# google-research/corenet

Measured on AMD Instinct MI355X. Metric: voxels/sec fwd+bwd @128^3, higher is better.
Workload: dtype bf16x3 (the convolutions of decoder stages 3-6 and the encoder's 3x3 convolutions -- forward of stages 4-5, data gradient of all -- multiply operands split into two bf16 terms: three bf16 MFMAs per product, fp32 accumulation, 16 mantissa bits, ~3e-6 relative per layer; tensors, everything else and t

## Files before the change

corenet_amd/_lib.py:

```python
from __future__ import annotations

import ctypes as C
import os
from typing import Optional

import torch as t

_HERE = os.path.dirname(os.path.abspath(__file__))
TOOLS_LIB_PATH = os.path.join(os.path.dirname(_HERE), "tools", "_build", "libcorenet_hip_tools.so")
PROBE_LIB_PATH = os.path.join(os.path.dirname(_HERE), "tools", "_build", "libcrn_probe.so")
LIB_PATH = os.environ.get("CORENET_HIP_LIB", TOOLS_LIB_PATH if os.environ.get("CRN_TOOLS_LIB") == "1" else
                          os.path.join(_HERE, "lib", "libcorenet_hip.so"))

c_i32p = C.POINTER(C.c_int32)
c_f32p = C.c_void_p
vp = C.c_void_p
i64 = C.c_int64
i32 = C.c_int
f32 = C.c_float
sz = C.c_size_t


class CrnTapBoxes(C.Structure):
  _fields_ = [("n_groups", C.c_int32), ("c_groups", C.c_int32), ("n_box", (C.c_int8 * 6) * 8),
              ("c_box", (C.c_int8 * 6) * 8)]


class CrnView(C.Structure):
  _fields_ = [("base", vp), ("B", C.c_int32), ("C", C.c_int32), ("D", C.c_int32),
              ("H", C.c_int32), ("W", C.c_int32), ("sB", i64), ("sC", i64),
              ("chan_off", vp), ("sD", C.c_int32), ("sH", C.c_int32), ("sW", C.c_int32)]


class CrnConvPlan(C.Structure):
  _fields_ = [(n, C.c_int32) for n in ("path", "msub", "nsub", "xstage", "dystage", "forced", "cc", "td", "th", "tw", "mw",
                                        "splits", "chunks", "vec_store", "balanced", "lds_bytes", "lds_budget")]


class CrnBf3Plan(C.Structure):
  _fields_ = [(n, C.c_int32) for n in ("kind", "nsub", "xmode", "ng", "slabs", "td", "th", "tw", "splits", "chunks", "per_split",
                                        "vec_store", "mode", "rowskip", "half_last", "lead", "n_groups", "c_groups", "nparts",
                                        "dmode", "tpw", "twt", "pipe", "inherit", "boxskip", "lds_bytes")]


BF3_KINDS = {0: "plain", 1: "half", 2: "ws"}
PLAN_PATHS = {1: "dense_cols", 2: "dense_rows", 3: "dense_wgrad", 4: "pointwise", 5: "generic"}


class CrnInTransform(C.Structure):
  _fields_ = [("scale", vp), ("shift", vp), ("pre_relu", C.c_int32), ("post_relu", C.c_int32)]


class CrnBnBwdFuse(C.Structure):
  _fields_ = [("x", vp), ("sB_x", i64), ("saved", vp), ("pre_relu", C.c_int32), ("ws", vp), ("ws_bytes", sz),
              ("dsum", vp), ("ndsum", C.c_int32), ("nparts", C.c_int32)]


class HipError(RuntimeError):
  pass


_SIGS = {
    "crn_conv_fwd": [C.POINTER(CrnView), C.POINTER(CrnInTransform), vp, i32, vp, i32,
                     C.POINTER(CrnView), i32, i32, i32, i32, i32, i32, i32, i32, vp, vp],
    "crn_conv_fwd_plan": [C.POINTER(CrnView), C.POINTER(CrnInTransform), vp, i32, vp, i32,
                          C.POINTER(CrnView), i32, i32, i32, i32, i32, i32, i32, i32, vp, C.POINTER(CrnConvPlan)],
    "crn_conv_wgrad_plan": [C.POINTER(CrnView), C.POINTER(CrnInTransform), C.POINTER(CrnView), vp, i32,
                            i32, i32, i32, i32, i32, i32, i32, vp, C.POINTER(CrnConvPlan)],
    "crn_conv_fwd_bf3": [C.POINTER(CrnView), C.POINTER(CrnInTransform), vp, i32, vp, i32,
                         C.POINTER(CrnView), i32, i32, i32, i32, i32, i32, i32, vp, vp],
    "crn_conv_fwd_bf3_slabs": [C.POINTER(CrnView), C.POINTER(CrnInTransform), vp, i32, vp, i32,
                               C.POINTER(CrnView), i32, i32, i32, i32, i32, i32, i32, vp, vp],
    "crn_conv_fwd_bf3_slabs_bnbwd": [C.POINTER(CrnView), C.POINTER(CrnInTransform), vp, i32, vp, i32,
                                     C.POINTER(CrnView), i32, i32, i32, i32, i32, i32, i32, vp, C.POINTER(CrnBnBwdFuse), vp],
    "crn_conv_fwd_bf3_slabs_stats": [C.POINTER(CrnView), C.POINTER(CrnInTransform), vp, i32, vp, i32,
                                     C.POINTER(CrnView), i32, i32, i32, i32, i32, i32, i32, vp, i32, vp, sz, C.POINTER(C.c_int), vp],
    "crn_batch_renorm_bwd_apply": [vp, i64, vp, i64, i32, i32, i64, i32, vp, vp, vp, vp, vp, i64, vp, vp, i32, vp, i32,
                                   vp, sz, i32, vp],
    "crn_conv_wgrad_bf3": [C.POINTER(CrnView), C.POINTER(CrnInTransform), C.POINTER(CrnView), vp, i32,
                           i32, i32, i32, i32, i32, i32, i32, vp],
    "crn_conv_wgrad_bf3_boxes": [C.POINTER(CrnView), C.POINTER(CrnInTransform), C.POINTER(CrnView), vp, i32,
                                 i32, i32, i32, i32, i32, i32, i32, vp, vp],
    "crn_conv_fwd_bf3_plan": [C.POINTER(CrnView), C.POINTER(CrnInTransform), vp, vp, i32, vp, i32,
                              C.POINTER(CrnView), i32, i32, i32, i32, i32, i32, i32, vp, vp, vp],
    "crn_conv_wgrad_bf3_plan": [C.POINTER(CrnView), C.POINTER(CrnInTransform), C.POINTER(CrnView), vp, i32,
                                i32, i32, i32, i32, i32, i32, i32, vp, vp],
    "crn_conv_wgrad": [C.POINTER(CrnView), C.POINTER(CrnInTransform), C.POINTER(CrnView), vp, i32,
                       i32, i32, i32, i32, i32, i32, i32, vp, vp],
    "crn_bf3_operands": [vp, vp, i32, i64, vp, vp],
    "crn_bf3_gather_image": [vp, vp, i32, vp, vp],
    "crn_convt_s2k7_fwd_bf3": [vp, i64, i32, i32, i32, i32, C.POINTER(CrnInTransform), vp, vp, vp, i64, i64, i32, vp],
    "crn_convt_s2k7_dgrad_bf3": [vp, i64, i64, i32, i32, i32, i32, i32, vp, vp, i64, i32, vp],
    "crn_convt_s2k7_c2_fwd_bf3": [vp, i64, i32, i32, i32, i32, C.POINTER(CrnInTransform), vp, vp, vp, i64, i64, i32, vp],
    "crn_convt_s2k7_c2_dgrad_bf3": [vp, i64, i64, i32, i32, i32, i32, i32, vp, vp, i64, i32, vp],
    "crn_convt_s2k7_wgrad_bf3": [vp, i64, i32, i32, i32, i32, C.POINTER(CrnInTransform), vp, i64, i64, i32, vp, i32, i32, vp, vp],
    "crn_convt_s2k7_ximage": [vp, i64, i32, i32, i32, i32, C.POINTER(CrnInTransform), vp, sz, vp],
    "crn_splitk_defer": [i32],
    "crn_splitk_reserve": [i64, vp],
    "crn_splitk_release": [vp],
    "crn_set_deterministic": [i32],
    "crn_roctx_push": [C.c_char_p],
    "crn_roctx_pop": [],
    "crn_comm_unique_id": [vp],
    "crn_comm_init": [vp, i32, i32, C.POINTER(vp)],
    "crn_comm_destroy": [vp],
    "crn_comm_info": [vp, C.POINTER(i32), C.POINTER(i32), C.POINTER(i32)],
    "crn_allreduce_f32": [vp, vp, i64, vp],
    "crn_broadcast_f32": [vp, vp, i64, i32, vp],
    "crn_conv_wgrad_1x1_bf3": [C.POINTER(CrnView), C.POINTER(CrnInTransform), C.POINTER(CrnView), vp, i32, i32, vp],
    "crn_conv_wgrad_2d_bf3": [C.POINTER(CrnView), C.POINTER(CrnInTransform), C.POINTER(CrnView), vp, i32, i32, i32, i32,
                              i32, i32, vp],
    "crn_conv2d_bf3": [C.POINTER(CrnView), C.POINTER(CrnInTransform), vp, i32, vp, i32, C.POINTER(CrnView),
                       i32, i32, i32, i32, i32, vp],
    "crn_copy_tiles_f32": [vp, vp, vp, vp, vp, i64, i32, vp],
    "crn_copy_mats_f32": [vp, vp, vp, i64, i32, vp],
    "crn_gather_f32": [vp, vp, vp, i64, vp],
    "crn_scatter_f32": [vp, vp, vp, i64, i32, vp],
    "crn_bias_grad": [vp, i32, i32, i64, i64, vp, i32, vp, sz, vp],
    "crn_batch_renorm_stats": [vp, i32, i32, i64, i64, i32, vp, vp, vp, vp, vp, f32, f32, i32,
                               vp, vp, vp, vp, sz, vp],
    "crn_batch_renorm_stats_tail": [vp, i32, i32, i64, i64, vp, vp, vp, vp, vp, f32, f32, i32, vp, vp, vp, vp, sz,
                                    vp, vp, vp, i64, vp, i64, vp, i64, i32, vp, i32, vp],
    "crn_batch_renorm_bwd_head": [vp, i64, vp, i64, vp, i64, vp, i64, vp, i64, i32, i32, i64, vp, vp, vp, vp, vp, i64,
                                  vp, vp, i32, vp, i32, vp, sz, vp, i32, vp],
    "crn_batch_renorm_bwd": [vp, i64, vp, i64, i32, i32, i64, i32, i32, vp, vp, vp, vp, vp, i64,
                             vp, vp, i32, vp, i32, vp, sz, vp],
    "crn_affine_add_relu": [vp, vp, vp, vp, vp, vp, i32, i32, i64, i64, i64, vp, i64, vp, i64, i32, vp],
    "crn_relu_bwd_add": [vp, vp, vp, i32, i32, i64, i64, i64, i64, vp, i64, vp],
    "crn_preprocess_caffe": [vp, i32, i32, i32, vp, vp],
    "crn_stem_conv_fwd": [vp, i32, i32, i32, vp, vp, vp, vp, sz, vp],
    "crn_stem_conv_wgrad": [vp, i32, i32, i32, vp, vp, vp],
    "crn_batch_renorm_finalize": [vp, i32, i32, C.c_double, vp, vp, vp, vp, vp, f32, f32, vp, vp, vp, vp],
    "crn_bn_relu_maxpool_fwd": [vp, vp, vp, i32, i32, i32, i32, vp, vp, vp],
    "crn_bn_relu_maxpool_bwd": [vp, vp, i32, i32, i32, i32, vp, vp],
    "crn_relu_mean_fwd": [vp, i32, i32, i64, i64, vp, vp],
    "crn_relu_mean_bwd": [vp, vp, i32, i32, i64, i64, vp, i64, i32, vp],
    "crn_linear_fwd": [vp, vp, vp, i32, i32, i32, vp, i32, vp],
    "crn_linear_bwd": [vp, vp, vp, i32, i32, i32, i32, vp, vp, vp, vp],
    "crn_stride2_gather": [vp, vp, i32, i32, i32, i32, i32, i32, vp],
    "crn_stride2_scatter": [vp, vp, i32, i32, i32, i32, i32, i32, vp],
    "crn_fill_offset_channels": [vp, i32, i64, i64, i32, vp, vp],
    "crn_decoder_inputs": [vp, vp, i32, i32, C.POINTER(C.c_float), vp, vp, vp],
    "crn_ray_sample_fwd": [vp, i64, i64, i64, i32, i32, i32, i32, vp, vp, vp, i64, i32, i32, i32, vp],
    "crn_ray_sample_bwd": [vp, i64, i32, i32, i32, i32, i32, vp, vp, vp, i64, i32, i32, i32, vp],
    "crn_ray_sample_fwd_idx": [vp, i64, i64, i64, i32, i32, i32, i32, vp, vp, vp, i64, i32, i32, i32, vp, vp],
    "crn_ray_project": [vp, vp, i32, i32, i32, i32, i32, i32, vp, vp],
    "crn_ray_sample_bwd_idx": [vp, i64, i32, i32, i32, i32, i32, vp, vp, i64, i32, i32, i32, vp],
    "crn_loss_fwd_bwd": [i32, vp, vp, vp, i32, i32, i64, vp, vp, f32, vp, sz, vp],
    "crn_argmax_confusion": [vp, vp, i32, i32, i64, vp, vp, vp],
    "crn_softmax_superres": [vp, i32, i32, i32, i32, i32, i32, vp, vp],
    "crn_eval_labels": [vp, vp, vp, i32, i32, i32, i32, i32, i32, i32, i32, vp, vp, vp, vp],
    "crn_eval_labels_cpu": [vp, vp, vp, i32, i32, i32, i32, i32, i32, i32, i32, vp, vp, vp, i32],
    "crn_adam_step": [vp, vp, vp, vp, i64, f32, f32, f32, f32, f32, i32, vp],
    "crn_adam_set_hyper": [vp, f32, f32, f32, f32, f32, i32, vp],
    "crn_adam_step_hyper": [vp, vp, vp, vp, i64, vp, vp],
    "crn_fill_voxels": [vp, vp, i32, i32, i32, i32, i32, vp, sz, vp],
    "crn_fill_voxels_strided": [vp, C.POINTER(i64), vp, C.POINTER(i64), i32, i32, i32, i32, i32, vp, sz, vp],
    "crn_fill_voxels_cpu": [vp, vp, i32, i32, i32, i32, i32, i32],
    "crn_marching_cubes_count": [vp, C.POINTER(i64), i32, i32, i32, i32, f32, vp, sz, vp, vp],
    "crn_marching_cubes_emit": [vp, C.POINTER(i64), i32, i32, i32, i32, f32, vp, vp, sz, vp, vp, vp, vp],
    "crn_marching_cubes_cpu": [vp, C.POINTER(i64), i32, i32, i32, i32, f32, vp, vp, vp, vp, vp, i32],
    "crn_box_filter": [vp, C.POINTER(i64), vp, i32, i32, i32, i32, i32, vp, sz, vp],
    "crn_box_filter_cpu": [vp, C.POINTER(i64), vp, i32, i32, i32, i32, i32, i32],
    "crn_render_bin": [vp, vp, i32, i32, i32, i32, i64, vp, vp, vp, vp],
    "crn_render_raster": [vp, vp, vp, vp, i32, vp, i32, i32, i32, i32, vp, vp, vp, vp, vp, vp],
    "crn_render_cpu": [vp, vp, vp, vp, i32, vp, i32, i32, i32, vp, i32],
    "crn_voxel_faces_count": [vp, i32, i32, i32, i32, vp, i32, vp, vp, vp, sz, vp, vp],
    "crn_voxel_faces_emit": [vp, i32, i32, i32, i32, vp, i32, vp, i32, vp, sz, vp, vp, vp, vp],
    "crn_voxel_faces_cpu": [vp, i32, i32, i32, i32, vp, i32, vp, vp, vp, i32, vp, vp, vp, vp, i32],
    "crn_sample_surface": [vp, vp, i32, i64, i64, C.c_uint32, vp, sz, vp, vp, vp, vp],
    "crn_sample_surface_cpu": [vp, vp, i32, i64, C.c_uint32, vp, vp, vp, i32],
    "crn_nearest": [vp, vp, vp, vp, i32, i64, i64, i64, vp, sz, vp, vp, vp],
# ... 140 lines not shown
```

corenet_amd/backend.py:

```python
from __future__ import annotations

import ctypes as C
from typing import Optional

import torch as t

from corenet_amd import _lib
from corenet_amd._lib import CrnInTransform, CrnView, ptr
from corenet_amd.views import View, space_to_depth_view, view_of

_DTYPE_CODE = {t.float32: 0, t.uint8: 1, t.int32: 2, t.float64: 3, t.int64: 4, t.int16: 5, t.int8: 6}


def _cview(v: View) -> CrnView:
  base = v.storage.data_ptr() + 4 * (v.offset - v.storage.storage_offset())
  c = v.__dict__.get("_crn")
  if c is None or c[0] != base:
    c = (base, CrnView(base, v.B, v.C, v.D, v.H, v.W, v.sB, v.sC, ptr(v.chan_off), v.sD, v.sH, v.sW))
    object.__setattr__(v, "_crn", c)
  return c[1]


class Transform:
  __slots__ = ("scale", "shift", "pre_relu", "post_relu")

  def __init__(self, scale: t.Tensor, shift: t.Tensor, pre_relu=False, post_relu=False):
    self.scale, self.shift = scale, shift
    self.pre_relu, self.post_relu = bool(pre_relu), bool(post_relu)


def _ctr(tr: Optional[Transform]):
  if tr is None:
    return None
  return C.byref(CrnInTransform(ptr(tr.scale), ptr(tr.shift), int(tr.pre_relu), int(tr.post_relu)))


_TAPBOXES = {}


def _ctapboxes(boxes):
  if not boxes or not (boxes[0] or boxes[1]):
    return None
  key = (tuple(boxes[0]), tuple(boxes[1]))
  tb = _TAPBOXES.get(key)
  if tb is None:
    tb = _lib.CrnTapBoxes()
    tb.n_groups, tb.c_groups = len(key[0]), len(key[1])
    for g, bx in enumerate(key[0]):
      for i, v in enumerate(bx): tb.n_box[g][i] = v
    for g, bx in enumerate(key[1]):
      for i, v in enumerate(bx): tb.c_box[g][i] = v
    _TAPBOXES[key] = tb
  return C.cast(C.pointer(tb), C.c_void_p)


class HipBackend:
  name = "hip"

  def __init__(self):
    self.lib = _lib.lib()
    self._ws = {}
    self._deterministic = False

  def workspace(self, key: str, nbytes: int, device) -> t.Tensor:
    w = self._ws.get((key, str(device)))
    if w is None or w.numel() < nbytes:
      w = t.empty(max(nbytes, 1), dtype=t.uint8, device=device)
      self._ws[(key, str(device))] = w
    return w

  def _bn_ws(self, Cn: int, device):
    n = self.lib.crn_batch_renorm_workspace_bytes(Cn)
    return self.workspace("bn@%x" % _lib.stream(), n, device), n

  def conv_fwd(self, x: View, tr: Optional[Transform], w: t.Tensor, npad: int,
               bias: Optional[t.Tensor], bias_sB: int, y: View, window, pad_lo,
               splits: int = 1, accumulate: bool = False, boxes=None, math: str = "fp32", wslab=None):
    if math == "bf16x3" and wslab is not None:
      self.lib.crn_conv_fwd_bf3_slabs(C.byref(_cview(x)), _ctr(tr), ptr(wslab), npad, ptr(bias), bias_sB,
                                      C.byref(_cview(y)), window[0], window[1], window[2],
                                      pad_lo[0], pad_lo[1], pad_lo[2], int(accumulate), _ctapboxes(boxes), _lib.stream())
      return
    if math == "bf16x3":
      self.lib.crn_conv_fwd_bf3(C.byref(_cview(x)), _ctr(tr), ptr(w), npad, ptr(bias), bias_sB,
                                C.byref(_cview(y)), window[0], window[1], window[2],
                                pad_lo[0], pad_lo[1], pad_lo[2], int(accumulate), _ctapboxes(boxes), _lib.stream())
      return
    self.lib.crn_conv_fwd(C.byref(_cview(x)), _ctr(tr), ptr(w), npad, ptr(bias), bias_sB,
                          C.byref(_cview(y)), window[0], window[1], window[2],
                          pad_lo[0], pad_lo[1], pad_lo[2], splits, int(accumulate), _ctapboxes(boxes),
                          _lib.stream())

  @staticmethod
  def _plan_dict(p) -> dict:
    d = {n: int(getattr(p, n)) for n, _ in p._fields_}
    d["path"] = _lib.PLAN_PATHS[d["path"]]
    return d

  def conv_fwd_plan(self, x: View, tr: Optional[Transform], w: t.Tensor, npad: int, bias: Optional[t.Tensor], bias_sB: int,
                    y: View, window, pad_lo, splits: int = 1, accumulate: bool = False, boxes=None) -> dict:
    p = _lib.CrnConvPlan()
    self.lib.crn_conv_fwd_plan(C.byref(_cview(x)), _ctr(tr), ptr(w), npad, ptr(bias), bias_sB, C.byref(_cview(y)),
                               window[0], window[1], window[2], pad_lo[0], pad_lo[1], pad_lo[2], splits, int(accumulate),
                               _ctapboxes(boxes), C.byref(p))
    return self._plan_dict(p)

  def conv_wgrad_plan(self, x: View, tr: Optional[Transform], dy: View, dw: t.Tensor, npad: int, window, pad_lo,
                      zero_first: bool = True, boxes=None) -> dict:
    p = _lib.CrnConvPlan()
    self.lib.crn_conv_wgrad_plan(C.byref(_cview(x)), _ctr(tr), C.byref(_cview(dy)), ptr(dw), npad, window[0], window[1],
                                 window[2], pad_lo[0], pad_lo[1], pad_lo[2], int(zero_first), _ctapboxes(boxes), C.byref(p))
    return self._plan_dict(p)

  def conv_fwd_bf3_plan(self, x: View, tr: Optional[Transform], w: Optional[t.Tensor], npad: int, bias: Optional[t.Tensor],
                        bias_sB: int, y: View, window, pad_lo, accumulate: bool = False, boxes=None, wslab=None, fuse=None) -> dict:
    p = _lib.CrnBf3Plan()
    self.lib.crn_conv_fwd_bf3_plan(C.byref(_cview(x)), _ctr(tr), None if wslab is not None else ptr(w), ptr(wslab), npad, ptr(bias),
                                   bias_sB, C.byref(_cview(y)), window[0], window[1], window[2], pad_lo[0], pad_lo[1], pad_lo[2],
                                   int(accumulate), _ctapboxes(boxes), None if fuse is None else C.addressof(fuse), C.addressof(p))
    d = {n: int(getattr(p, n)) for n, _ in p._fields_}
    d["kind"] = _lib.BF3_KINDS[d["kind"]]
    return d

  def conv_wgrad_bf3_plan(self, x: View, tr: Optional[Transform], dy: View, dw: t.Tensor, npad: int, window, pad_lo,
                          zero_first: bool = True, boxes=None) -> dict:
    p = _lib.CrnBf3Plan()
    self.lib.crn_conv_wgrad_bf3_plan(C.byref(_cview(x)), _ctr(tr), C.byref(_cview(dy)), ptr(dw), npad, window[0], window[1],
                                     window[2], pad_lo[0], pad_lo[1], pad_lo[2], int(zero_first), _ctapboxes(boxes), C.addressof(p))
    return {n: int(getattr(p, n)) for n, _ in p._fields_}

  def conv_fwd_stats(self, x: View, tr: Optional[Transform], wslab: t.Tensor, npad: int, bias, bias_sB: int, y: View, window,
                     pad_lo, boxes, Cn: int, pre_relu: bool) -> int:
    ws, n = self._bn_ws(Cn, y.storage.device)
    parts = C.c_int(0)
    self.lib.crn_conv_fwd_bf3_slabs_stats(C.byref(_cview(x)), _ctr(tr), ptr(wslab), npad, ptr(bias), bias_sB,
                                          C.byref(_cview(y)), window[0], window[1], window[2], pad_lo[0], pad_lo[1], pad_lo[2],
                                          0, _ctapboxes(boxes), int(pre_relu), ptr(ws), n, C.byref(parts), _lib.stream())
    return parts.value

  def conv_dgrad_bn_bwd(self, dyv: View, wslab: t.Tensor, npad: int, gv: View, g: t.Tensor, window, pad_lo, boxes,
                        x, sB_x, B, Cn, S, pre_relu, gamma, scale, shift, saved, dx, sB_dx, dgamma, dbeta,
                        dsum=None, ndsum=0) -> bool:
    ws, n = self._bn_ws(Cn, x.device)
    f = _lib.CrnBnBwdFuse(ptr(x), sB_x, ptr(saved), int(pre_relu), ptr(ws), n, ptr(dsum), int(ndsum), 0)
    self.lib.crn_conv_fwd_bf3_slabs_bnbwd(C.byref(_cview(dyv)), None, ptr(wslab), npad, None, 0, C.byref(_cview(gv)),
                                          window[0], window[1], window[2], pad_lo[0], pad_lo[1], pad_lo[2], 0,
                                          _ctapboxes(boxes), C.byref(f), _lib.stream())
    if f.nparts <= 0:
      return False
    self.lib.crn_batch_renorm_bwd_apply(ptr(x), sB_x, ptr(g), Cn * S, B, Cn, S, int(pre_relu), ptr(gamma),
                                        ptr(scale), ptr(shift), ptr(saved), ptr(dx), sB_dx, ptr(dgamma), ptr(dbeta),
                                        0, ptr(dsum), int(ndsum), ptr(ws), n, f.nparts, _lib.stream())
    return True

  def splitk_defer(self, on: bool = True):
    self.lib.crn_splitk_defer(int(on))

  def set_deterministic(self, on: bool = True):
    self.lib.crn_set_deterministic(int(on))
    self._deterministic = bool(on)

  def splitk_reserve(self, stream: t.cuda.Stream, floats: int = 0):
    self.lib.crn_splitk_reserve(int(floats), stream.cuda_stream)

  def splitk_release(self, stream: t.cuda.Stream):
    self.lib.crn_splitk_release(stream.cuda_stream)
    for k in [k for k in self._ws if k[0] == "bn@%x" % stream.cuda_stream]:
      del self._ws[k]

  def bf3_operands(self, packed: t.Tensor, table, out: t.Tensor):
    desc, blocks = table
    self.lib.crn_bf3_operands(ptr(packed), ptr(desc), desc.shape[0], blocks, ptr(out), _lib.stream())

  def bf3_gather_image(self, src: t.Tensor, table: t.Tensor, out: t.Tensor, host_table=None):
    self.lib.crn_bf3_gather_image(ptr(src), ptr(table), table.shape[0], ptr(out), _lib.stream())

  def convt_par_fwd(self, x: t.Tensor, tr: Optional[Transform], wimg: t.Tensor, bias: Optional[t.Tensor], y: t.Tensor, cout: int,
                    host_table=None, resident: bool = False):
    B, cin, D, H, W = x.shape
    assert cin == 16 and x[0].is_contiguous() and y[0].is_contiguous() and tuple(y.shape[2:]) == (2 * D, 2 * H, 2 * W)
    fn = self.lib.crn_convt_s2k7_c2_fwd_bf3 if resident else self.lib.crn_convt_s2k7_fwd_bf3
    fn(ptr(x), x.stride(0), B, D, H, W, _ctr(tr), ptr(wimg), ptr(bias), ptr(y), y.stride(0), y.stride(1), cout, _lib.stream())

  def convt_par_dgrad(self, dy: t.Tensor, cout: int, wimg: t.Tensor, dx: t.Tensor, accumulate: bool = False, host_table=None,
                      resident: bool = False):
    B, cin, D, H, W = dx.shape
    assert cin == 16 and dx[0].is_contiguous() and dy[0].is_contiguous() and tuple(dy.shape[2:]) == (2 * D, 2 * H, 2 * W)
    fn = self.lib.crn_convt_s2k7_c2_dgrad_bf3 if resident else self.lib.crn_convt_s2k7_dgrad_bf3
    fn(ptr(dy), dy.stride(0), dy.stride(1), cout, B, D, H, W, ptr(wimg), ptr(dx), dx.stride(0), int(accumulate), _lib.stream())

  def conv2d_bf3(self, x: View, tr: Optional[Transform], wop: t.Tensor, npad: int, bias: Optional[t.Tensor],
                 bias_sB: int, y: View, window, pad_lo, accumulate: bool = False):
    assert window[0] == 1 and pad_lo[0] == 0
    self.lib.crn_conv2d_bf3(C.byref(_cview(x)), _ctr(tr), ptr(wop), npad, ptr(bias), bias_sB, C.byref(_cview(y)),
                            window[1], window[2], pad_lo[1], pad_lo[2], int(accumulate), _lib.stream())

  def _ximage(self, xp: int, sB: int, B: int, D: int, H: int, W: int, tr: Optional[Transform], alloc) -> t.Tensor:
    nb = self.lib.crn_convt_s2k7_ximage_bytes(B, D, H, W)
    img = alloc(nb)
    self.lib.crn_convt_s2k7_ximage(xp, sB, B, D, H, W, _ctr(tr), ptr(img), nb, _lib.stream())
    return img

  def convt_ximage(self, x: t.Tensor, tr: Optional[Transform], img: Optional[t.Tensor] = None) -> Optional[t.Tensor]:
    if self._deterministic:
      return None
    B, cin, D, H, W = x.shape
    assert cin == 16 and x[0].is_contiguous()
    return self._ximage(ptr(x), x.stride(0), B, D, H, W, tr,
                        lambda nb: img if img is not None and img.numel() >= nb else t.empty(nb, dtype=t.uint8, device=x.device))

  def _wgrad_ct_par(self, x: View, tr: Optional[Transform], dy: View, dw: t.Tensor, npad: int, zero_first: bool,
                    ximg: Optional[t.Tensor]) -> bool:
    assert x.chan_off is None and x.C == 16 and x.sW == 1 and x.sH == x.W and x.sD == x.H * x.W and x.sC == x.D * x.H * x.W, x
    ds, C8 = dy.storage, dy.C // 8
    assert ds.dim() == 5 and dy.C == 8 * C8 and tuple(ds.shape[2:]) == (2 * x.D, 2 * x.H, 2 * x.W) and ds[0, 0].is_contiguous(), dy
    ref = space_to_depth_view(view_of(ds).channels(0, C8), (2, 2, 2), parity_major=True)
    assert all(getattr(dy, f) == getattr(ref, f) for f in ("offset", "B", "C", "D", "H", "W", "sB", "sC", "sD", "sH", "sW")), dy
    assert dy.chan_off is ref.chan_off, "dy is not the parity-major view"
    xp = x.storage.data_ptr() + 4 * (x.offset - x.storage.storage_offset())
    if ximg is None and not self._deterministic:
      ximg = self._ximage(xp, x.sB, x.B, x.D, x.H, x.W, tr, lambda nb: self.workspace("ct_ximg", nb, ds.device))
    rc = self.lib._crn_convt_s2k7_wgrad_bf3(xp, x.sB, x.B, x.D, x.H, x.W, _ctr(tr), ds.data_ptr(), ds.stride(0), ds.stride(1), C8,
                                            ptr(dw), npad, int(zero_first), ptr(ximg), _lib.stream())
    if rc not in (0, -1):
      raise _lib.HipError(f"crn_convt_s2k7_wgrad_bf3 failed with status {rc}")
    return rc == 0

  def conv_wgrad(self, x: View, tr: Optional[Transform], dy: View, dw: t.Tensor, npad: int,
                 window, pad_lo, zero_first: bool = True, boxes=None, math: str = "fp32", ximg: Optional[t.Tensor] = None):
    if math == "bf16x3_1x1":
      self.lib.crn_conv_wgrad_1x1_bf3(C.byref(_cview(x)), _ctr(tr), C.byref(_cview(dy)), ptr(dw), npad, int(zero_first),
                                      _lib.stream())
      return
    if math == "bf16x3_2d":
      self.lib.crn_conv_wgrad_2d_bf3(C.byref(_cview(x)), _ctr(tr), C.byref(_cview(dy)), ptr(dw), npad, window[1],
                                     window[2], pad_lo[1], pad_lo[2], int(zero_first), _lib.stream())
      return
    if math == "ct_par":
      if self._wgrad_ct_par(x, tr, dy, dw, npad, zero_first, ximg):
        return
      math = "bf16x3"
    if math == "bf16x3":
      self.lib.crn_conv_wgrad_bf3_boxes(C.byref(_cview(x)), _ctr(tr), C.byref(_cview(dy)), ptr(dw), npad,
                                        window[0], window[1], window[2], pad_lo[0], pad_lo[1], pad_lo[2],
                                        int(zero_first), _ctapboxes(boxes), _lib.stream())
      return
    if math == "stem":
      rc = self.lib._crn_stem_conv_wgrad(x.storage.data_ptr() + 4 * x.offset, x.B, 2 * x.H, 2 * x.W,
                                         dy.storage.data_ptr() + 4 * dy.offset, ptr(dw), _lib.stream())
      if rc == 0:
        return
      if rc != -1:
        raise _lib.HipError(f"crn_stem_conv_wgrad failed with status {rc}")
    self.lib.crn_conv_wgrad(C.byref(_cview(x)), _ctr(tr), C.byref(_cview(dy)), ptr(dw), npad,
                            window[0], window[1], window[2], pad_lo[0], pad_lo[1], pad_lo[2],
# ... 259 lines not shown
```

corenet_amd/csrc/conv_e2d.hip:

```cpp
#include "conv_kernels.h"
#include "bf3_common.h"
#include <algorithm>
#include <cstdlib>

namespace {
using namespace crnk;

struct E2dGeom {
  crnView x, y;
  crnInTransform tr;
  const void* wop;
  const float* bias;
  int bias_sB;
  int ntn;
  int nblk;
  int ph, pw;
  int tilesH, tilesW;
  int nchunks, chunks_per_split;
  int tab;
  int mode;
  int dbg;
  long long* stamps;
};

constexpr int kOpFields = 7;

__global__ __launch_bounds__(256) void bf3_operands_kernel(const float* packed, const long long* desc, int nlayers,
                                                           char* out) {
  int lo = 0, hi = nlayers - 1;
  while (lo < hi) {
    const int mid = (lo + hi + 1) >> 1;
    if (desc[mid * kOpFields + 5] <= (long long)blockIdx.x) lo = mid; else hi = mid - 1;
  }
  const long long* d = desc + lo * kOpFields;
  const int Cin = (int)d[2], T = (int)d[3], Npad = (int)d[4];
  if (d[6] > 0) {
    const int KHW = (int)d[6], kd = T / KHW, TP = (KHW + 3) & ~3;
    const long long entries = (long long)((Cin + 7) >> 3) * kd * TP * Npad;
    const long long e = ((long long)blockIdx.x - d[5]) * 256 + threadIdx.x;
    if (e >= entries) return;
    const int n = (int)(e % Npad);
    long long r = e / Npad;
    const int tp = (int)(r % TP); r /= TP;
    const int zd = (int)(r % kd);
    const int chunk = (int)(r / kd);
    float v[8];
#pragma unroll
    for (int j = 0; j < 8; ++j) {
      const int c = chunk * 8 + j;
      v[j] = (c < Cin && tp < KHW) ? packed[d[0] + ((long long)c * T + zd * KHW + tp) * Npad + n] : 0.f;
    }
    bf16x8 h, l;
    split8(v, h, l);
    bf16x8* dst = reinterpret_cast<bf16x8*>(out + (d[1] + e) * 32);
    dst[0] = h;
    dst[1] = l;
    return;
  }
  const int ntn = Npad >> 4;
  const long long entries = (long long)(Cin >> 5) * T * ntn * 64;
  const long long e = ((long long)blockIdx.x - d[5]) * 256 + threadIdx.x;
  if (e >= entries) return;
  const int lane = (int)(e & 63);
  const long long rest = e >> 6;
  const int ntile = (int)(rest % ntn);
  const int kg = (int)(rest / ntn);
  const int cbg = kg / T, t = kg - cbg * T;
  const int kk = lane >> 4, i16 = lane & 15;
  const float* src = packed + d[0] + ((long long)(cbg * 32 + kk * 8) * T + t) * Npad + ntile * 16 + i16;
  float v[8];
#pragma unroll
  for (int j = 0; j < 8; ++j) v[j] = src[(long long)j * T * Npad];
  bf16x8 h, l;
  split8(v, h, l);
  bf16x8* dst = reinterpret_cast<bf16x8*>(out + (d[1] + e) * 32);
  dst[0] = h;
  dst[1] = l;
}

constexpr unsigned kOOB = 0x80000000u;

template <int N>
__device__ __forceinline__ void wait_vm(f32x4& a, f32x4& b) {
  asm volatile("s_waitcnt vmcnt(%2)" : "+v"(a), "+v"(b) : "n"(N));
}

template <int T, int CB, int TW>
__global__ __launch_bounds__(256, 2) void conv_e2d_kernel(E2dGeom g) {
  constexpr int KW = T == 9 ? 3 : 1;
  constexpr int TH = 64 / TW, PH = TH + KW - 1, PW = TW + KW - 1, NPOS = PH * PW;
  constexpr int NPA = T == 9 ? 128 : 64;
  constexpr int KS = CB * T;
  constexpr int NPL = T == 9 ? 16 : 8;
  constexpr int PS = NPA + 4;
  constexpr int PLANE = CB * 4 * PS;
  static_assert(T == 9 ? CB == 1 : CB == 4, "thread -> patch element mapping");
  extern __shared__ __attribute__((aligned(16))) char smem[];
  float* tscale = reinterpret_cast<float*>(smem);
  float* tshift = tscale + g.tab;
  bf16x8* Abuf = reinterpret_cast<bf16x8*>(smem + (size_t)g.tab * 8);

  const long long t_entry = (long long)__builtin_amdgcn_s_memtime();
  crn_kernargs_now(g.x.base, g.x.B, g.x.C, g.x.H, g.x.W, g.x.sB, g.x.sC, g.x.sH, g.y.base, g.y.C, g.y.sB, g.y.sC, g.y.sH,
               g.tr.scale, g.tr.shift, g.tr.pre_relu, g.tr.post_relu, g.wop, g.bias, g.bias_sB, g.ntn, g.nblk, g.ph,
               g.pw, g.tilesH, g.tilesW, g.nchunks, g.chunks_per_split, g.tab, g.mode, g.dbg, g.stamps, gridDim.x);
  if (g.dbg & 1) return;
  const bool stamp = (g.dbg & 16) && blockIdx.x == 0 && blockIdx.y == 0 && blockIdx.z == 0 && threadIdx.x == 0;
  auto mark = [&](int i) { if (stamp) g.stamps[i] = (long long)__builtin_amdgcn_s_memtime() - t_entry; };
  mark(0);
  const int tid = threadIdx.x, lane = tid & 63, wave = tid >> 6;
  const int i16 = lane & 15, kk = lane >> 4;
  int tile = xcd_remap(blockIdx.x, gridDim.x);
  const int twi = tile % g.tilesW; tile /= g.tilesW;
  const int thi = tile % g.tilesH; tile /= g.tilesH;
  const int b = tile;
  const int split = blockIdx.z;
  const int cbeg = split * g.chunks_per_split, cend = min(cbeg + g.chunks_per_split, g.nchunks);
  const int ch0 = cbeg * CB * 32;
  const bool has_tr = g.tr.scale != nullptr;

  const crn_rsrc xrs = make_rsrc(g.x.base + (int64_t)b * g.x.sB);
  const crn_rsrc wrs = make_rsrc(reinterpret_cast<const float*>(g.wop));

  const int kk8 = tid & 3;
  unsigned poff[2];
  bool pin[2] = {false, false};
  int h0 = 0, w0 = 0, p0 = 0;
  if constexpr (T == 9) {
    h0 = thi * TH; w0 = twi * TW;
#pragma unroll
    for (int p = 0; p < 2; ++p) {
      const int q = (tid >> 2) + 64 * p;
      const int r = q / PW, c = q - r * PW;
      const int gh = h0 - g.ph + r, gw = w0 - g.pw + c;
      pin[p] = q < NPOS && gh >= 0 && gh < g.x.H && gw >= 0 && gw < g.x.W;
      poff[p] = pin[p] ? (unsigned)(gh * g.x.sH + gw) * 4u : kOOB;
    }
  } else {
    p0 = twi * 64;
    poff[0] = (unsigned)(p0 + 4 * ((tid >> 2) & 15)) * 4u;
    poff[1] = 0;
  }
  const unsigned sC4 = (unsigned)g.x.sC * 4u;

  float pf[T == 9 ? 16 : 1];
  f32x4 pv[T == 9 ? 1 : 8];
  auto patch_issue = [&](int chunk) {
    if constexpr (T == 9) {
      const unsigned oob = chunk < cend ? 0u : kOOB;
      const unsigned cbase = (unsigned)(chunk * 32 + kk8 * 8) * sC4;
#pragma unroll
      for (int p = 0; p < 2; ++p)
#pragma unroll
        for (int j = 0; j < 8; ++j) crn_bload(pf[p * 8 + j], xrs, (poff[p] + cbase + (unsigned)j * sC4) | oob);
    } else {
      const int cbg = chunk * CB + wave;
      const unsigned oob = (chunk < cend && cbg < g.nblk) ? 0u : kOOB;
      const unsigned cbase = (unsigned)(cbg * 32 + kk8 * 8) * sC4;
#pragma unroll
      for (int j = 0; j < 8; ++j) crn_bload4(pv[j], xrs, (poff[0] + cbase + (unsigned)j * sC4) | oob);
// ... 394 lines not shown
#pragma unroll
    for (int qt = 0; qt < 2; ++qt) asm volatile("s_waitcnt vmcnt(0)" : "+v"(ra[qt][0]), "+v"(ra[qt][1]), "+v"(el[qt]), "+v"(er[qt]));
#pragma unroll
    for (int nt = 0; nt < 2; ++nt) asm volatile("s_waitcnt vmcnt(0)" : "+v"(rb[nt][0]), "+v"(rb[nt][1]));
  };
  auto tf = [&](float a, int qt, bool valid) -> float {
    if (!has_tr) return a;
    if (g.pre_relu) a = fmaxf(a, 0.f);
    a = a * sc[qt] + sh[qt];
    if (g.post_relu) a = fmaxf(a, 0.f);
    return valid ? a : 0.f;
  };
  int step = kbeg + wave;
  issue(step);
  for (; step < kend; step += 4) {
    wait_all();
    bf16x8 ah[6], al[6], bh[2], bl[2];
#pragma unroll
    for (int qt = 0; qt < 2; ++qt) {
      float u[10];
      u[0] = tf(el[qt], qt, (vmask >> (2 + qt)) & 1u);
#pragma unroll
      for (int j = 0; j < 8; ++j) u[1 + j] = tf(ra[qt][j >> 2][j & 3], qt, (vmask >> qt) & 1u);
      u[9] = tf(er[qt], qt, (vmask >> (4 + qt)) & 1u);
#pragma unroll
      for (int zw = 0; zw < 3; ++zw) {
        float v[8];
#pragma unroll
        for (int j = 0; j < 8; ++j) v[j] = u[j + zw];
        split8(v, ah[qt * 3 + zw], al[qt * 3 + zw]);
      }
    }
#pragma unroll
    for (int nt = 0; nt < 2; ++nt) {
      float v[8];
#pragma unroll
      for (int j = 0; j < 8; ++j) v[j] = rb[nt][j >> 2][j & 3];
      split8(v, bh[nt], bl[nt]);
    }
    issue(step + 4);
#pragma unroll
    for (int nt = 0; nt < 2; ++nt) {
#pragma unroll
      for (int mt = 0; mt < 6; ++mt) acc[mt][nt] = __builtin_amdgcn_mfma_f32_16x16x32_bf16(ah[mt], bh[nt], acc[mt][nt], 0, 0, 0);
#pragma unroll
      for (int mt = 0; mt < 6; ++mt) acc[mt][nt] = __builtin_amdgcn_mfma_f32_16x16x32_bf16(ah[mt], bl[nt], acc[mt][nt], 0, 0, 0);
#pragma unroll
      for (int mt = 0; mt < 6; ++mt) acc[mt][nt] = __builtin_amdgcn_mfma_f32_16x16x32_bf16(al[mt], bh[nt], acc[mt][nt], 0, 0, 0);
    }
  }
  wait_all();
#pragma unroll
  for (int mt = 0; mt < 6; ++mt)
#pragma unroll
    for (int nt = 0; nt < 2; ++nt) red[wave][mt * 2 + nt][lane] = acc[mt][nt];
  __syncthreads();
#pragma unroll
  for (int j = 0; j < 3; ++j) {
    const int tile = wave * 3 + j;
    const f32x4 v = red[0][tile][lane] + red[1][tile][lane] + red[2][tile][lane] + red[3][tile][lane];
    const int mt = tile >> 1, nt = tile & 1, qt = mt / 3, zw = mt - 3 * qt;
    const int n = n0 + 16 * nt + i16;
#pragma unroll
    for (int r = 0; r < 4; ++r) {
      const int q = q0 + 16 * qt + 4 * kk + r;
      if (q < 3 * g.C && n < g.N) atomicAdd(g.dw + (long long)(3 * q + zw) * g.Npad + n, v[r]);
    }
  }
}

bool dense_2d(const crnView& v) {
  return v.chan_off == nullptr && v.sW == 1 && v.sH == v.W && (v.D == 1 || v.sD == v.H * v.W) && (v.sC & 3) == 0 &&
         (v.sB & 3) == 0 && (((uintptr_t)v.base) & 15) == 0;
}

}

extern "C" int crn_bf3_operands(const float* packed, const int64_t* desc, int nlayers, int64_t total_blocks, void* out,
                                crnStream stream) {
  CRN_ENTRY(stream);
  if (!packed || !desc || !out || nlayers < 1 || total_blocks < 1 || total_blocks > 0x7fffffff) return CRN_EINVAL;
  hipLaunchKernelGGL(bf3_operands_kernel, dim3((unsigned)total_blocks), dim3(256), 0, (hipStream_t)stream, packed,
                     reinterpret_cast<const long long*>(desc), nlayers, reinterpret_cast<char*>(out));
  CRN_CHECK_LAUNCH();
  return CRN_OK;
}

namespace {
long long* g_stamps = nullptr;
template <int T, int CB, int TW>
int launch_e2d(const E2dGeom& g, dim3 grid, size_t lds, hipStream_t st) {
  return crn_launch(conv_e2d_kernel<T, CB, TW>, grid, dim3(256), lds, st, g);
}
}

extern "C" int crn_conv2d_bf3(const crnView* x, const crnInTransform* tr, const void* wop, int Npad, const float* bias,
                              int bias_sB, const crnView* y, int kh, int kw, int ph, int pw, int accumulate,
                              crnStream stream) {
  if (!x || !y || !wop || x->B != y->B || x->B < 1) return CRN_EINVAL;
  if (!dense_2d(*x) || !dense_2d(*y)) return CRN_EINVAL;
  if ((x->C & 31) || (y->C & 63) || Npad != y->C) return CRN_EINVAL;
  if (x->D != y->D || x->H != y->H || x->W != y->W) return CRN_EINVAL;
  const bool k3 = kh == 3 && kw == 3, k1 = kh == 1 && kw == 1;
  if (!k3 && !k1) return CRN_EINVAL;
  if (k1 && (ph || pw)) return CRN_EINVAL;
  const int64_t S = (int64_t)x->D * x->H * x->W;
  if (S * x->C * 4 >= ((int64_t)1 << 31)) return CRN_EINVAL;
  hipStream_t st = (hipStream_t)stream;
  int rcf;
  const bool armed = crn_splitk_begin(st, &rcf);
  if (rcf != CRN_OK) return rcf;
  E2dGeom g{};
  g.x = *x; g.y = *y;
  if (tr) g.tr = *tr; else g.tr = crnInTransform{nullptr, nullptr, 0, 0};
  g.wop = wop; g.bias = bias; g.bias_sB = bias_sB;
  g.ntn = Npad / 16; g.nblk = x->C / 32; g.ph = ph; g.pw = pw;
#ifdef CRN_TOOLS
  static const bool want_stamps = getenv("CRN_E2D_DBG") && (atoi(getenv("CRN_E2D_DBG")) & 16);
  if (want_stamps) {
    if (!g_stamps) CRN_HIP(hipMalloc(&g_stamps, 32 * sizeof(long long)));
    g.stamps = g_stamps;
    g.dbg = 16;
  }
#endif
  int TW = 16, CB = 1;
  int64_t tiles;
  if (k3) {
    if (x->D != 1 || ph < 0 || ph > 2 || pw < 0 || pw > 2) return CRN_EINVAL;
    TW = (x->W % 16 == 0) ? 16 : 8;
    const int TH = 64 / TW;
    if (x->W % TW || x->H % TH) return CRN_EINVAL;
    g.tilesW = x->W / TW; g.tilesH = x->H / TH;
    tiles = (int64_t)g.tilesW * g.tilesH;
    g.nchunks = g.nblk;
  } else {
    if (S % 64) return CRN_EINVAL;
    CB = 4;
    g.tilesW = (int)(S / 64); g.tilesH = 1;
    tiles = g.tilesW;
    g.nchunks = (g.nblk + CB - 1) / CB;
  }
  const int64_t base_blocks = tiles * x->B * (y->C / 64);
  constexpr int kFill = 256;
  int splits = 1;
  while (base_blocks * splits < kFill && splits * 2 <= g.nchunks && splits < 16) splits *= 2;
  g.chunks_per_split = (g.nchunks + splits - 1) / splits;
  splits = (g.nchunks + g.chunks_per_split - 1) / g.chunks_per_split;
  g.tab = g.tr.scale ? g.chunks_per_split * CB * 32 : 0;
  const crnView yreal = *y;
  float* scratch = nullptr;
  if (splits > 1) {
    scratch = crn_splitk_scratch((size_t)splits * x->B * y->C * S, st);
    if (!scratch) return CRN_ENOMEM;
    g.y = crn_splitk_scratch_view(yreal, scratch);
    g.mode = 3;
  } else {
    g.mode = accumulate ? 1 : 0;
  }
  const size_t plane_bytes = (size_t)(k3 ? 4 * (128 + 4) : 16 * (64 + 4)) * 16;
  const size_t lds = (size_t)g.tab * 8 + 4 * plane_bytes;
  if (lds > 160 * 1024) return CRN_EINVAL;
  const dim3 grid((unsigned)(tiles * x->B), (unsigned)(y->C / 64), (unsigned)splits);
  int rc;
  if (k1) rc = launch_e2d<1, 4, 16>(g, grid, lds, st);
  else if (TW == 16) rc = launch_e2d<9, 1, 16>(g, grid, lds, st);
  else rc = launch_e2d<9, 1, 8>(g, grid, lds, st);
// ... 69 lines not shown
```

corenet_amd/csrc/conv_igemm.hip:

```cpp
#include "conv_kernels.h"
#include <algorithm>
#include <cstring>
#include <cstdio>
#include <cstdlib>

namespace {
using namespace crnk;

struct PwGeom {
  const float* x; float* y; const float* w; const float* bias;
  crnInTransform tr;
  int B, C, N, Npad, S;
  int64_t xsB, ysB;
  int64_t ysC, ysP;
  int bias_sB, mode;
  int splits, cps;
  long long* stamps;
};

constexpr int kPwBN = 32;
constexpr int kPwTab = 2048;
template <int NS>
__global__ __launch_bounds__(256) void pointwise_fwd_kernel(PwGeom g) {
  constexpr int BM = 64, BN = NS * 16, KC = 64, SA = BM + 16, SB = BN + 16;
  constexpr int NRA = KC / 16;
  __shared__ __attribute__((aligned(16))) float ldsA[KC * SA];
  __shared__ __attribute__((aligned(16))) float ldsB[KC * SB];
  crn_kernargs_now(g.x, g.y, g.w, g.bias, g.tr.scale, g.tr.shift, g.tr.pre_relu, g.tr.post_relu, g.B, g.C, g.N, g.Npad,
                   g.S, g.xsB, g.ysB, g.ysC, g.ysP, g.bias_sB, g.mode, g.splits, g.cps);
  const long long t_entry = (long long)__builtin_amdgcn_s_memtime();
  const long long r_entry = (long long)__builtin_amdgcn_s_memrealtime();
  const int tid = threadIdx.x, lane = tid & 63, wave = tid >> 6;
  const int i16 = lane & 15, kk = lane >> 4;
  const int m0 = blockIdx.x * BM, n0 = blockIdx.y * BN;
  const bool stamp = g.stamps && blockIdx.x == 0 && blockIdx.y == 0 && blockIdx.z == 0 && tid == 0;
  int nmark = 0;
  auto mark = [&]() { if (stamp && nmark < 30) g.stamps[nmark] = (long long)__builtin_amdgcn_s_memtime() - t_entry; ++nmark; };
  mark();
  const int split = blockIdx.z / g.B, b = blockIdx.z - split * g.B;
  const int cbeg = split * g.cps, cend = min(g.C, cbeg + g.cps);
  const float* xb = g.x + (int64_t)b * g.xsB;
  const int ka = tid >> 4, ca = (tid & 15) * 4;
  constexpr int BQ = BN / 4, BROWS = 256 / BQ, NRB = KC / BROWS;
  const int kb = tid / BQ, cb = (tid % BQ) * 4;
  const bool a_ok = (m0 + ca) < g.S;
  const bool b_ok = (n0 + cb) < g.Npad;
  extern __shared__ float pw_tables[];
  const bool has_tr = g.tr.scale != nullptr;
  float* tsc = pw_tables; float* tsh = pw_tables + g.cps;
  constexpr unsigned kOOBo = 0x80000000u;
  constexpr int NL = NRA + NRB;
  const crn_rsrc xrs = crnk::make_rsrc(xb);
  const crn_rsrc wrs = crnk::make_rsrc(g.w);
  f32x4 ra[2][NRA], rb[2][NRB];
  auto issue = [&](int c0, f32x4 (&pa_)[NRA], f32x4 (&pb_)[NRB]) {
#pragma unroll
    for (int q = 0; q < NRA; ++q) {
      const int c_a = c0 + ka + q * 16;
      const unsigned off = (a_ok && c_a < cend) ? (unsigned)(c_a * g.S + m0 + ca) * 4u : kOOBo;
      crnk::crn_bload4(pa_[q], xrs, off);
    }
#pragma unroll
    for (int q = 0; q < NRB; ++q) {
      const int c_b = c0 + kb + q * BROWS;
      const unsigned off = (b_ok && c_b < cend) ? (unsigned)(c_b * g.Npad + n0 + cb) * 4u : kOOBo;
      crnk::crn_bload4(pb_[q], wrs, off);
    }
  };
  auto wait_slot = [&](f32x4 (&pa_)[NRA], f32x4 (&pb_)[NRB]) {
#pragma unroll
    for (int q = 0; q < NRA; ++q) asm volatile("s_waitcnt vmcnt(%1)" : "+v"(pa_[q]) : "n"(NL));
#pragma unroll
    for (int q = 0; q < NRB; ++q) asm volatile("s_waitcnt vmcnt(%1)" : "+v"(pb_[q]) : "n"(NL));
  };
  auto xform = [&](f32x4 v, int c) -> f32x4 {
    if (has_tr && a_ok && c < cend) {
      const float sc = tsc[c - cbeg], sh = tsh[c - cbeg];
#pragma unroll
      for (int i = 0; i < 4; ++i) {
        float t = v[i];
        if (g.tr.pre_relu) t = fmaxf(t, 0.f);
        t = t * sc + sh;
        if (g.tr.post_relu) t = fmaxf(t, 0.f);
        v[i] = t;
      }
    }
    return v;
  };
  f32x4 acc[NS];
#pragma unroll
  for (int ns = 0; ns < NS; ++ns) acc[ns] = (f32x4){0.f, 0.f, 0.f, 0.f};
  issue(cbeg, ra[0], rb[0]);
  issue(cbeg + KC, ra[1], rb[1]);
  mark();
  if (has_tr)
    for (int c = tid; c < cend - cbeg; c += 256) { tsc[c] = g.tr.scale[cbeg + c]; tsh[c] = g.tr.shift[cbeg + c]; }
  auto step = [&](int c0, f32x4 (&pa_)[NRA], f32x4 (&pb_)[NRB]) {
    wait_slot(pa_, pb_);
    mark();
    __syncthreads();
#pragma unroll
    for (int q = 0; q < NRA; ++q) *reinterpret_cast<f32x4*>(ldsA + (ka + q * 16) * SA + ca) = xform(pa_[q], c0 + ka + q * 16);
#pragma unroll
    for (int q = 0; q < NRB; ++q) *reinterpret_cast<f32x4*>(ldsB + (kb + q * BROWS) * SB + cb) = pb_[q];
    __syncthreads();
    mark();
    issue(c0 + 2 * KC, pa_, pb_);
    const float* pa = ldsA + kk * SA + wave * 16 + i16;
    const float* pb = ldsB + kk * SB + i16;
#pragma unroll
    for (int ks = 0; ks < KC / 4; ++ks) {
      const float a = pa[ks * 4 * SA];
      float bv[NS];
#pragma unroll
      for (int ns = 0; ns < NS; ++ns) bv[ns] = pb[ks * 4 * SB + ns * 16];
#pragma unroll
      for (int ns = 0; ns < NS; ++ns) acc[ns] = __builtin_amdgcn_mfma_f32_16x16x4f32(a, bv[ns], acc[ns], 0, 0, 0);
    }
    mark();
  };
  for (int c0 = cbeg; c0 < cend; c0 += 2 * KC) {
    step(c0, ra[0], rb[0]);
    if (c0 + KC < cend) step(c0 + KC, ra[1], rb[1]);
  }
#pragma unroll
  for (int sl = 0; sl < 2; ++sl) {
#pragma unroll
    for (int q = 0; q < NRA; ++q) asm volatile("s_waitcnt vmcnt(0)" : "+v"(ra[sl][q]));
#pragma unroll
    for (int q = 0; q < NRB; ++q) asm volatile("s_waitcnt vmcnt(0)" : "+v"(rb[sl][q]));
  }
  const int m = m0 + wave * 16 + kk * 4;
  if (m < g.S) {
#pragma unroll
    for (int ns = 0; ns < NS; ++ns) {
      const int n = n0 + ns * 16 + i16;
      if (n < g.N) {
        const float bsv = (g.bias && split == 0) ? g.bias[(int64_t)b * g.bias_sB + n] : 0.f;
        float* dst = g.y + (int64_t)(split * g.B + b) * g.ysB + (int64_t)n * g.ysC + (int64_t)m * g.ysP;
        f32x4 v = acc[ns] + bsv;
        if (g.ysP == 1) {
          if (g.mode == 1) v += *reinterpret_cast<const f32x4*>(dst);
          *reinterpret_cast<f32x4*>(dst) = v;
        } else {
#pragma unroll
          for (int i = 0; i < 4; ++i) dst[i * g.ysP] = g.mode == 1 ? dst[i * g.ysP] + v[i] : v[i];
        }
      }
    }
  }
  if (stamp) {
    g.stamps[31] = (long long)__builtin_amdgcn_s_memtime() - t_entry;
    g.stamps[30] = (long long)__builtin_amdgcn_s_memrealtime() - r_entry;
  }
}

constexpr int kDenseB = 8;
__global__ __launch_bounds__(256) void dense_cols_kernel(const float* x, int64_t xsB, int64_t xsC, crnInTransform tr,
                                                         const float* w, int Npad, int N, int C, int B,
                                                         const float* bias, int bias_sB, float* y, int64_t ysB,
                                                         int64_t ysC, int accumulate) {
  extern __shared__ float xs[];
  __shared__ float red[3][kDenseB][64];
  const int lane = threadIdx.x & 63, wave = threadIdx.x >> 6;
  const int n = blockIdx.x * 64 + lane;
  const int cq = (C + 3) >> 2, cbeg = wave * cq, cend = min(C, cbeg + cq);
  const bool col = n < N;
  float wv[32];
#pragma unroll
  for (int u = 0; u < 32; ++u) wv[u] = (col && cbeg + u < cend) ? w[(int64_t)(cbeg + u) * Npad + n] : 0.f;
  for (int i = threadIdx.x; i < B * C; i += blockDim.x) {
    const int b = i / C, c = i - b * C;
    float v = x[b * xsB + c * xsC];
    if (tr.scale) {
      if (tr.pre_relu) v = fmaxf(v, 0.f);
      v = v * tr.scale[c] + tr.shift[c];
      if (tr.post_relu) v = fmaxf(v, 0.f);
    }
    xs[i] = v;
  }
  __syncthreads();
  float acc[kDenseB];
#pragma unroll
  for (int b = 0; b < kDenseB; ++b) acc[b] = 0.f;
  for (int c = cbeg; c < cend; c += 32) {
    if (c > cbeg) {
#pragma unroll
      for (int u = 0; u < 32; ++u) wv[u] = (col && c + u < cend) ? w[(int64_t)(c + u) * Npad + n] : 0.f;
    }
#pragma unroll
    for (int u = 0; u < 32; ++u)
#pragma unroll
      for (int b = 0; b < kDenseB; ++b)
        if (b < B && c + u < cend) acc[b] += xs[b * C + c + u] * wv[u];
  }
  if (wave) {
#pragma unroll
    for (int b = 0; b < kDenseB; ++b) red[wave - 1][b][lane] = acc[b];
  }
  __syncthreads();
  if (wave || !col) return;
#pragma unroll
  for (int b = 0; b < kDenseB; ++b)
    if (b < B) {
      float* d = y + b * ysB + n * ysC;
      const float v = ((acc[b] + red[0][b][lane]) + (red[1][b][lane] + red[2][b][lane])) +
                      (bias ? bias[(int64_t)b * bias_sB + n] : 0.f);
      *d = accumulate ? *d + v : v;
    }
}
__global__ __launch_bounds__(256) void dense_rows_kernel(const float* x, int64_t xsB, int64_t xsC, const float* w,
                                                         int Npad, int N, int C, const float* bias, int bias_sB,
                                                         float* y, int64_t ysB, int64_t ysC, int accumulate,
                                                         int cps) {
  __shared__ float red[4][8];
  const int b = blockIdx.y, n0 = blockIdx.x * 8;
  const int lane = threadIdx.x & 63, wave = threadIdx.x >> 6;
  float acc[8];
#pragma unroll
  for (int j = 0; j < 8; ++j) acc[j] = 0.f;
  const float* xb = x + b * xsB;
  const int cbeg = blockIdx.z * cps, cend = min(C, cbeg + cps);
#pragma unroll 4
  for (int c = cbeg + threadIdx.x; c < cend; c += 256) {
    const float xv = xb[c * xsC];
    const f32x4 w0 = *reinterpret_cast<const f32x4*>(w + (int64_t)c * Npad + n0);
    const f32x4 w1 = *reinterpret_cast<const f32x4*>(w + (int64_t)c * Npad + n0 + 4);
#pragma unroll
    for (int j = 0; j < 4; ++j) { acc[j] += xv * w0[j]; acc[4 + j] += xv * w1[j]; }
  }
#pragma unroll
  for (int j = 0; j < 8; ++j) {
    const float v = crn_wave_sum(acc[j]);
    if (lane == 0) red[wave][j] = v;
  }
  __syncthreads();
  if (threadIdx.x < 8 && n0 + (int)threadIdx.x < N) {
    const int n = n0 + threadIdx.x;
// ... 155 lines not shown
      return CRN_OK;
    }
  }
  if (kd * kh * kw == 1 && pd == 0 && ph == 0 && pw == 0 && splits <= 1 && plain_view(*x) && flat_out_view(*y) &&
      Sx == (int64_t)y->D * y->H * y->W && (Sx & 3) == 0 && (((uintptr_t)w) & 15) == 0 &&
      (int64_t)x->C * Sx * 4 < ((int64_t)1 << 31) && (int64_t)x->C * Npad * 4 < ((int64_t)1 << 31) &&
      (!has_scale || x->C <= kPwTab)) {
    s->path = CRN_PLAN_POINTWISE;
    s->pw_splits = 1; s->pw_cps = s->pw_cps_whole = (x->C + 63) & ~63;
    constexpr int pw_blocks = 256, pw_fill = 512, pw_minc = 128;
    const int64_t blocks = crn_cdiv(Sx, 64) * crn_cdiv(y->C, kPwBN) * (int64_t)x->B;
    if (splits < 1 && blocks < pw_blocks && x->C >= 2 * pw_minc) {
      int sp = (int)std::min<int64_t>(std::min<int64_t>(x->C / pw_minc, 16), crn_cdiv(pw_fill, blocks));
      if (sp > 1) {
        const int cps = (crn_cdiv(x->C, sp) + 31) & ~31;
        sp = crn_cdiv(x->C, cps);
        if (sp > 1) { s->pw_splits = sp; s->pw_cps = cps; }
        s->pw_cps_whole = (x->C + 31) & ~31;
      }
    }
    return CRN_OK;
  }
  s->path = CRN_PLAN_GENERIC;
  static const int kM[4] = {8, 4, 2, 1};
  static const int kN[3] = {4, 2, 1};
  const int xmode = vec_view(*x) ? 1 : ((x->sW == 2 && (x->W & 1) == 0) ? 2 : 0);
  g_stage_unit = xmode == 2 ? 2 : 4;
  const int lead = xmode == 1 ? vec_lead(pw) : (xmode == 2 ? ((pw % 2) + 2) % 2 : -1);
  constexpr double kSplitPenalty = 20000.0;
  constexpr int kSplitFill = 512;
  FwdCfg best{}; bool have = false; double best_cost = 1e300; int best_splits = 1;
  for (int mi = 0; mi < 4; ++mi)
    for (int ni = 0; ni < 3; ++ni) {
      if (kN[ni] > 1 && kN[ni] * 16 > Npad) continue;
      if (kM[mi] * kN[ni] > 8) continue;
      FwdCfg c;
      if (!fwd_cfg(kM[mi], kN[ni], y->B, x->C, Npad, y->D, y->H, y->W, kd, kh, kw, lead, &c)) continue;
      const int T = kd * kh * kw, nchunks = crn_cdiv(x->C, c.CC), NB = kN[ni] * 16;
      const int TD = c.tsd, TH = c.tsh * c.mh, TW = c.tsw * c.mw;
      const double patch = (double)c.CC * (TD + kd - 1) * (TH + kh - 1) * patch_width(TW, kw, lead);
      const double slots = (lead >= 0 ? patch / g_stage_unit / 256 * (g_stage_unit == 4 ? 450.0 : 400.0) : patch / 256 * 350.0) +
                           (double)c.CC * T * NB / 4 / 256 * 300.0;
      const double chunk_work = (double)kM[mi] * kN[ni] * (c.CC / 4) * T * 32.0 * 1.3 + slots;
      for (int sp = 1; sp <= (splits < 1 ? std::min(nchunks, 64) : 1); sp *= 2) {
        if (sp > 1 && c.blocks * (sp / 2) >= kSplitFill) break;
        const int cps = crn_cdiv(nchunks, sp);
        const double bpc = std::max(1.0, std::ceil((double)c.blocks * sp / 256.0));
        double cost = bpc * cps * chunk_work + cps * std::ceil(bpc / 2.0) * 9000.0 + (sp > 1 ? kSplitPenalty : 0.0);
        if (cost < best_cost) { best_cost = cost; best = c; have = true; best_splits = sp; }
      }
    }
  bool forced = false;
  int xvec = lead >= 0 ? xmode : 0;
  if (!have && xvec) {
    xvec = 0;
    for (int mi = 0; mi < 4 && !have; ++mi) {
      FwdCfg c;
      if (fwd_cfg(kM[mi], 1, y->B, x->C, Npad, y->D, y->H, y->W, kd, kh, kw, -1, &c)) { best = c; have = true; forced = true; }
    }
  }
  if (!have) return CRN_EINVAL;
  s->cfg = best; s->xvec = xvec; s->lead = lead; s->forced = forced;
  s->nchunks = crn_cdiv(x->C, best.CC);
  if (splits < 1) {
    splits = forced ? (best.blocks >= 192 ? 1 : (int)std::min<int64_t>(std::min(s->nchunks, 16), crn_cdiv(256, best.blocks)))
                    : best_splits;
  }
  if (splits > s->nchunks) splits = s->nchunks;
  s->splits = crn_cdiv(s->nchunks, crn_cdiv(s->nchunks, splits));
  return CRN_OK;
}

}

static long long* g_pw_stamps = nullptr;
#ifdef CRN_TOOLS
extern "C" int crn_pw_debug_stamps(long long* out32) {
  if (!g_pw_stamps) return CRN_EINVAL;
  CRN_HIP(hipDeviceSynchronize());
  CRN_HIP(hipMemcpy(out32, g_pw_stamps, 32 * sizeof(long long), hipMemcpyDeviceToHost));
  return CRN_OK;
}
#endif
extern "C" int crn_conv_fwd(const crnView* x, const crnInTransform* tr, const float* w, int Npad,
                            const float* bias, int bias_sB, const crnView* y,
                            int kd, int kh, int kw, int pd, int ph, int pw,
                            int splits, int accumulate, const crnTapBoxes* boxes, crnStream stream) {
  const int rca = fwd_check_args(x, w, Npad, y, kd, kh, kw, boxes);
  if (rca != CRN_OK) return rca;
  hipStream_t st = (hipStream_t)stream;
  int rcf;
  const bool armed = crn_splitk_begin(st, &rcf);
  if (rcf != CRN_OK) return rcf;
  FwdSel sel;
  const int rcs = fwd_select(x, tr, w, Npad, y, kd, kh, kw, pd, ph, pw, splits, &sel);
  if (rcs != CRN_OK) return rcs;
  const int64_t Sx = (int64_t)x->D * x->H * x->W;
  if (sel.path == CRN_PLAN_DENSE_COLS) {
    const crnInTransform trv = tr ? *tr : crnInTransform{nullptr, nullptr, 0, 0};
    hipLaunchKernelGGL(dense_cols_kernel, dim3((unsigned)crn_cdiv(y->C, 64)), dim3(256), (size_t)x->B * x->C * 4, st,
                       x->base, x->sB, x->sC, trv, w, Npad, y->C, x->C, x->B, bias, bias_sB, y->base, y->sB, y->sC,
                       accumulate);
    CRN_CHECK_LAUNCH();
    return CRN_OK;
  }
  if (sel.path == CRN_PLAN_DENSE_ROWS) {
    const int zs = sel.zs;
    if (zs > 1 && !accumulate)
      CRN_HIP(hipMemset2DAsync(y->base, (size_t)y->sB * 4, 0, (size_t)y->C * 4, (size_t)x->B, st));
    hipLaunchKernelGGL(dense_rows_kernel, dim3((unsigned)crn_cdiv(y->C, 8), (unsigned)x->B, (unsigned)zs), dim3(256), 0, st,
                       x->base, x->sB, x->sC, w, Npad, y->C, x->C, bias, bias_sB, y->base, y->sB, y->sC, accumulate,
                       crn_cdiv(x->C, zs));
    CRN_CHECK_LAUNCH();
    return CRN_OK;
  }
  if (sel.path == CRN_PLAN_POINTWISE) {
    PwGeom p{};
    p.x = x->base; p.y = y->base; p.w = w; p.bias = bias;
    p.tr = tr ? *tr : crnInTransform{nullptr, nullptr, 0, 0};
    p.B = x->B; p.C = x->C; p.N = y->C; p.Npad = Npad; p.S = (int)Sx;
    p.xsB = x->sB; p.ysB = y->sB; p.bias_sB = bias_sB; p.mode = accumulate ? 1 : 0;
    p.ysC = y->sC; p.ysP = y->sW;
    p.splits = 1; p.cps = sel.pw_cps_whole;
    const int64_t ytot = (int64_t)y->B * y->C * Sx;
    float* scratch = nullptr;
    if (sel.pw_splits > 1 && (scratch = crn_splitk_scratch((size_t)sel.pw_splits * ytot, st)) != nullptr) {
      p.splits = sel.pw_splits; p.cps = sel.pw_cps;
      p.y = scratch; p.ysB = (int64_t)y->C * Sx; p.ysC = Sx; p.ysP = 1; p.mode = 0;
    }
#ifdef CRN_TOOLS
    static const bool want_stamps = getenv("CRN_PW_STAMPS") != nullptr;
#else
    constexpr bool want_stamps = false;
#endif
    static long long* pw_stamps = nullptr;
    if (want_stamps) {
      if (!pw_stamps) CRN_HIP(hipMalloc(&pw_stamps, 32 * sizeof(long long)));
      CRN_HIP(hipMemsetAsync(pw_stamps, 0, 32 * sizeof(long long), st));
      p.stamps = pw_stamps;
      g_pw_stamps = pw_stamps;
    }
    dim3 grid((unsigned)crn_cdiv(Sx, 64), (unsigned)crn_cdiv(y->C, kPwBN), (unsigned)(x->B * p.splits));
    const size_t tab_bytes = p.tr.scale ? (size_t)2 * p.cps * sizeof(float) : 0;
    hipLaunchKernelGGL(pointwise_fwd_kernel<kPwBN / 16>, grid, dim3(256), tab_bytes, st, p);
    CRN_CHECK_LAUNCH();
    return p.splits > 1 ? crn_splitk_finish(*y, scratch, p.splits, accumulate, armed, st) : CRN_OK;
  }
  const FwdCfg& best = sel.cfg;
  const int xvec = sel.xvec, lead = sel.lead;
  splits = sel.splits;
  ConvGeom g{};
  g.x = *x; g.y = *y;
  if (tr) g.tr = *tr; else g.tr = crnInTransform{nullptr, nullptr, 0, 0};
  g.w = w; g.bias = bias; g.Npad = Npad; g.bias_sB = bias_sB;
  g.lead = xvec ? lead : 0;
  g.kd = kd; g.kh = kh; g.kw = kw; g.pd = pd; g.ph = ph; g.pw = pw + g.lead; g.T = kd * kh * kw;
  g.mw = best.mw; g.mh = best.mh; g.nsh = best.tsh; g.nsw = best.tsw;
  g.TD = best.tsd; g.TH = best.tsh * best.mh; g.TW = best.tsw * best.mw;
  g.PD = g.TD + kd - 1; g.PH = g.TH + kh - 1; g.PW = patch_width(g.TW, kw, xvec ? lead : -1);
  g.PS = g.PD * g.PH * g.PW; g.PSP = pad16mod32(g.PS);
  g.tilesD = crn_cdiv(y->D, g.TD); g.tilesH = crn_cdiv(y->H, g.TH); g.tilesW = crn_cdiv(y->W, g.TW);
  const int NSUB = best.NSUB, CC = best.CC;
  g.CC = CC; g.WSP = pad16mod32(g.T * NSUB * 16);
  g.nchunks = sel.nchunks;
  g.chunks_per_split = crn_cdiv(g.nchunks, splits);
  g.mode = splits > 1 ? 2 : (accumulate ? 1 : 0);
  g.lg2 = ilog2_ceil(g.PH * g.PW); g.npass = xvec ? 0 : stage_passes(CC * g.PD, g.PH * g.PW);
  g.magic_PW = magic20(g.PW); g.magic_PD = magic20(g.PD); g.magic_T = magic20(g.T);
  if (xvec) {
    g.plu = g.PH * g.PW / g_stage_unit; g.pw4 = g.PW / g_stage_unit; g.nunits = CC * g.PD * g.plu;
    g.magic_PLU = magic20(g.plu); g.magic_PW4 = magic20(g.pw4);
  }
  const crnView yreal = *y;
  const int64_t ytot = (int64_t)y->B * y->C * y->D * y->H * y->W;
  float* scratch = g.mode == 2 ? crn_splitk_scratch((size_t)splits * ytot, st) : nullptr;
  if (scratch) {
    g.mode = 3;
    g.y = crn_splitk_scratch_view(yreal, scratch);
  }
  y = &g.y;
  if (g.mode == 2 && !accumulate) {
    hipLaunchKernelGGL(zero_view_kernel, dim3((unsigned)std::min<int64_t>(crn_cdiv(ytot, 256), 4096)),
                       dim3(256), 0, st, yreal);
    CRN_CHECK_LAUNCH();
  }
  dim3 grid((unsigned)(g.tilesD * g.tilesH * g.tilesW * y->B), (unsigned)crn_cdiv(Npad, NSUB * 16),
            (unsigned)splits);
  const size_t lds_bytes = best.lds;
  g.vec_store = fwd_vec_store(*y, g.mw, g.mode) ? 1 : 0;
  if (boxes) {
    if (boxes->n_groups > 0 && y->C % boxes->n_groups == 0) { g.n_groups = boxes->n_groups; memcpy(g.n_box, boxes->n_box, sizeof(g.n_box)); }
    if (boxes->c_groups > 0 && x->C % boxes->c_groups == 0) { g.c_groups = boxes->c_groups; memcpy(g.c_box, boxes->c_box, sizeof(g.c_box)); }
  }
  int rc = CRN_EINVAL;
#define CRN_FWD_CASE(M, N) if (best.MSUB == M && NSUB == N) rc = crn_launch_fwd_##M##_##N(g, xvec, grid, lds_bytes, st);
  CRN_FWD_CONFIGS(CRN_FWD_CASE)
#undef CRN_FWD_CASE
  if (rc == CRN_OK && g.mode == 3) rc = crn_splitk_finish(yreal, scratch, splits, accumulate, armed, st);
  return rc;
}

namespace {
struct WgCand { int TD, TH, TW, RSUB, NSUB, CC, PW, PSP, POSP; double cost; size_t lds; };

bool wg_cand(int TD, int TH, int TW, int RSUB, int NSUB, int Cin, int Npad, int kd, int kh, int kw, int xlead,
             int dvec, size_t lds_budget, WgCand* out) {
  const int T = kd * kh * kw, NB = NSUB * 16, npos = TD * TH * TW;
  if (npos > 512 || RSUB * NSUB > 8 || (NSUB > 1 && NB > Npad)) return false;
  if ((xlead >= 0 || dvec) && (TW & 3)) return false;
  if (dvec == 1 ? (int64_t)NB * npos / 4 > 256 * NV
                : dvec == 2 ? (int64_t)NB * npos / 2 > 256 * NVX : stage_passes(NB, npos) > DREG) return false;
  const int PDp = TD + kd - 1, PH = TH + kh - 1, PW = patch_width(TW, kw, xlead), plane = PH * PW;
  int CC = std::min(std::min(std::max(1, (64 * RSUB) / T), Cin), 64);
  auto staged = [&](int cc) {
    return xlead >= 0 ? (int64_t)cc * PDp * plane / 4 <= 256 * NVX : stage_passes(cc * PDp, plane) <= PREG;
  };
  while (CC > 1 && !staged(CC)) --CC;
  if (!staged(CC)) return false;
  const int PSP = xlead >= 0 ? pad16mod32(PDp * plane) : PDp * plane + 1;
  const int POSP = npos + 4;
  const size_t lds = ((size_t)CC * PSP + (size_t)NB * POSP + 2 * kChTab) * 4;
  if (lds > lds_budget) return false;
  const int rows = CC * T;
  if (rows > 64 * RSUB) return false;
  const double mfma = (double)RSUB * NSUB * (npos / 4.0) * 32.0;
  const double xslots = xlead >= 0 ? (double)CC * PDp * plane / 4 / 256 * 450.0 : (double)CC * PDp * plane / 256 * 350.0;
  const double dslots = dvec == 1 ? (double)NB * npos / 4 / 256 * 300.0
                                  : dvec == 2 ? (double)NB * npos / 2 / 256 * 300.0 : (double)NB * npos / 256 * 300.0;
  const double useful = (double)rows * std::min(NB, Npad) * npos;
  *out = WgCand{TD, TH, TW, RSUB, NSUB, CC, PW, PSP, POSP, (mfma + xslots + dslots + 800.0) / useful, lds};
  return true;
}
}

namespace {
int wgrad_check_args(const crnView* x, const crnView* dy, const float* dw, int Npad, int kd, int kh, int kw) {
  if (!x || !dy || !dw || Npad <= 0 || (Npad & 15) || x->B != dy->B) return CRN_EINVAL;
  if (kd * kh * kw > 512) return CRN_EINVAL;
  return CRN_OK;
}
bool wgrad_dense(const crnView* x, const crnView* dy, int T) {
  return T == 1 && one_position(*x) && one_position(*dy) && dy->C >= 1024;
}

struct WgSel {
  WgCand best;
  int xlead, dvec;
  int ntiles, cblocks, nblocks;
  int splits, tiles_per_split;
  bool balanced;
};

int wg_select(const crnView* x, const crnView* dy, int Npad, int kd, int kh, int kw, int pw, const crnTapBoxes* boxes,
              WgSel* s) {
  const int T = kd * kh * kw;
  g_stage_unit = 4;
  const int Dy = dy->D, Hy = dy->H, Wy = dy->W;
  const int TWc = Wy >= 16 ? 16 : ((Wy + 3) & ~3);
  int xlead = vec_view(*x) ? vec_lead(pw) : -1;
  int dvec = vec_view(*dy) ? 1 : ((dy->sW == 2 && dy->chan_off != nullptr && (dy->W & 1) == 0) ? 2 : 0);
  WgCand best{}; bool have = false;
  auto consider = [&](int TD, int TH, int RSUB, int NSUB, size_t budget) {
    WgCand c;
    if (!wg_cand(std::min(TD, Dy), std::min(TH, Hy), TWc, RSUB, NSUB, x->C, Npad, kd, kh, kw, xlead, dvec, budget, &c))
      return false;
    if (RSUB > 1 && c.CC * T <= 32 * RSUB) return false;
    if (!have || c.cost < best.cost) { best = c; have = true; }
    return true;
  };
  auto search = [&]() {
    static const int kTD[4] = {4, 3, 2, 1};
    static const int kTH[6] = {16, 8, 6, 4, 2, 1};
    for (int tdi = 0; tdi < 4; ++tdi)
      for (int thi = 0; thi < 6; ++thi)
        for (int NSUB = 4; NSUB >= 1; NSUB >>= 1)
          for (int RSUB = 8; RSUB >= 1; RSUB >>= 1) consider(kTD[tdi], kTH[thi], RSUB, NSUB, kLdsBudget);
  };
  search();
  if (!have && (xlead >= 0 || dvec)) { xlead = -1; dvec = 0; search(); }
  if (!have) return CRN_EINVAL;
  if (xlead < 0) dvec = 0;
  if (xlead < 0 || !dvec) {
// ... 161 lines not shown
```

corenet_amd/model/conv_geometry.py:

```python
from __future__ import annotations

import dataclasses
from typing import Tuple

import numpy as np


def pad16(n: int) -> int:
  return (n + 15) // 16 * 16


@dataclasses.dataclass
class Geom:
  window: Tuple[int, int, int]
  pad_lo: Tuple[int, int, int]
  index: np.ndarray
  cin: int
  nout: int
  npad: int
  n_boxes: Tuple = ()
  c_boxes: Tuple = ()

  @property
  def taps(self) -> int:
# ... 194 lines not shown


MAT_LDS = 8448


def mat_index(parts):
  descs, rest = [], []
  for part in parts:
    off, idx, cols, grows = part
    idx2 = np.asarray(idx, np.int64).reshape(-1, cols)
    rows = idx2.shape[0]
    gr = grows or rows
    ng = rows // gr
    idx3 = idx2.reshape(ng, gr, cols)
    v = idx3 >= 0
    R, N = int(v[0, :, 0].sum()), int(v[0, 0, :].sum())
    ok = R > 0 and N > 0 and R * N > 1 and bool(v[:, :R, :N].all()) and int(v.sum()) == ng * R * N
    if ok:
      base = int(idx3[0, 0, 0])
      rs = int(idx3[0, 1, 0]) - base if R > 1 else 0
      cs = int(idx3[0, 0, 1]) - base if N > 1 else 0
      gs = int(idx3[1, 0, 0]) - base if ng > 1 else 0
      pred = (base + np.arange(ng)[:, None, None] * gs + np.arange(R)[None, :, None] * rs + np.arange(N)[None, None, :] * cs)
      ok = bool((pred == idx3[:, :R, :N]).all()) and (abs(rs) == 1 or cs == 1)
    if not ok:
      rest.append(part)
      continue
    if abs(rs) == 1 and R > 1:
      nb, na = R, N
      f0 = base if rs == 1 else base - (R - 1)
      p0 = off if rs == 1 else off + (R - 1) * cols
      fa, pa, pb = cs, 1, (cols if rs == 1 else -cols)
    else:
      nb, na = N, R
      f0, p0 = base, off
      fa, pa, pb = rs, cols, 1
    fg, pg = gs, gr * cols
    bstep = nb if nb <= 128 else 64
    for b0 in range(0, nb, bstep):
      B = min(bstep, nb - b0)
      for a0 in range(0, na, 64):
        A = min(64, na - a0)
        gstep = max(1, MAT_LDS // (A * (B | 1))) if (B == nb and ng > 1) else 1
        g0 = np.arange(0, ng, gstep)
        G_ = np.minimum(gstep, ng - g0)
        d = np.zeros((len(g0), 16), np.int64)
        d[:, 0], d[:, 1], d[:, 2] = A, B, G_
        d[:, 3] = f0 + g0 * fg + a0 * fa + b0
        d[:, 4], d[:, 5] = fa, fg
        d[:, 6] = p0 + g0 * pg + a0 * pa + b0 * pb
        d[:, 7], d[:, 8], d[:, 9] = pa, pb, pg
        magic = lambda q: 0 if q == 1 else ((1 << 32) + q - 1) // q
        d[:, 10], d[:, 11], d[:, 12] = magic(A * B), magic(B), magic(A)
        descs.append(d)
  desc = np.concatenate(descs) if descs else np.zeros((0, 16), np.int64)
  assert np.abs(desc[:, :10]).max(initial=0) < 2 ** 31 and (desc[:, 2] * desc[:, 0] * (desc[:, 1] | 1) <= MAT_LDS).all()
  return desc.astype(np.uint32).view(np.int32), rest


def operand_eligible(g: Geom) -> bool:
  return (g.window in ((1, 1, 1), (1, 3, 3)) and g.cin % 32 == 0 and g.nout % 64 == 0 and g.npad == g.nout
          and not g.n_boxes and not g.c_boxes)


def operand_entries(g: Geom) -> int:
  return (g.cin // 32) * g.taps * (g.npad // 16) * 64


def slab_entries(g: Geom) -> int:
  khw = g.window[1] * g.window[2]
  return ((g.cin + 7) // 8) * g.window[0] * ((khw + 3) // 4 * 4) * g.npad


def operand_table(layers):
  rows, blocks = [], 0
  for layer in layers:
    src, dst, g = layer[:3]
    slab = len(layer) > 3 and layer[3]
    rows.append((src, dst, g.cin, g.taps, g.npad, blocks, g.window[1] * g.window[2] if slab else 0))
    blocks += ((slab_entries(g) if slab else operand_entries(g)) + 255) // 256
  return np.asarray(rows, dtype=np.int64).reshape(-1, 7), blocks


def _ct_table(rows_of_step):
  tab, off16 = [], 0
  for rows, entry in rows_of_step:
    hi0, lo0 = off16, off16 + rows * 128
    for zi in range(rows):
      for kk in range(4):
        for col in range(32):
          e = (zi * 4 + kk) * 32 + col
          tab.append(list(entry(zi, kk, col)) + [hi0 + e, lo0 + e])
    off16 += rows * 256
  return np.asarray(tab, np.int32), off16 * 16 + 4096


def convt_par_fwd_table(wshape, wofs: int = 0):
  Cc, N, ks = wshape[0], wshape[1], wshape[2]
  assert Cc == 16 and ks == 7 and N <= 16
  steps = []
  for pp in range(4):
    rd, rh = pp >> 1, pp & 1
    for ch in range(2):
      for zd in range(3 + rd):
        def entry(zh, kk, col, rd=rd, rh=rh, ch=ch, zd=zd):
          rw, n = col >> 4, col & 15
          kd, kh, kw = 5 - 2 * zd + rd, 5 - 2 * zh + rh, 5 - 2 * kk + rw
          if n >= N or kw < 0:
            return [-1] * 8
          return [wofs + (((ch * 8 + j) * N + n) * ks + kd) * ks * ks + kh * ks + kw for j in range(8)]
        steps.append((3 + rh, entry))
  return _ct_table(steps)


def convt_par_dgrad_table(wshape, wofs: int = 0):
  Cc, N, ks = wshape[0], wshape[1], wshape[2]
  assert Cc == 16 and ks == 7 and N <= 16
  steps = []
  for pp in range(4):
    rd, rh = pp >> 1, pp & 1
    for nh in range((N + 7) // 8):
      for zd in range(1 - rd, 4):
        def entry(zi, kk, col, rd=rd, rh=rh, nh=nh, zd=zd):
          rw, c = col >> 4, col & 15
          zh = 1 - rh + zi
          kd, kh, kw = 2 * zd - 1 + rd, 2 * zh - 1 + rh, 2 * kk - 1 + rw
          if kw < 0:
            return [-1] * 8
          return [(wofs + ((c * N + nh * 8 + j) * ks + kd) * ks * ks + kh * ks + kw) if nh * 8 + j < N else -1 for j in range(8)]
        steps.append((3 + rh, entry))
  return _ct_table(steps)


def convt_res_fwd_table(wshape, wofs: int = 0):
  Cc, N, ks = wshape[0], wshape[1], wshape[2]
  assert Cc == 16 and ks == 7 and N == 2
  tab = []
  for c in range(2):
    for zd in range(4):
      for zh in range(4):
        for kk in range(4):
          for col in range(16):
            rd, rh, rw, n = col >> 3, (col >> 2) & 1, (col >> 1) & 1, col & 1
            kd, kh, kw = 5 - 2 * zd + rd, 5 - 2 * zh + rh, 5 - 2 * kk + rw
            e = ((c * 4 + zd) * 4 + zh) * 64 + kk * 16 + col
            if min(kd, kh, kw) < 0:
              src = [-1] * 8
            else:
              src = [wofs + (((c * 8 + j) * N + n) * ks + kd) * ks * ks + kh * ks + kw for j in range(8)]
            tab.append(src + [e, 2048 + e])
  return np.asarray(tab, np.int32), 2 * 2048 * 16


def convt_res_dgrad_table(wshape, wofs: int = 0):
  Cc, N, ks = wshape[0], wshape[1], wshape[2]
  assert Cc == 16 and ks == 7 and N <= 2
  tab = []
  for rd in range(2):
    for zd in range(4):
      for zh in range(4):
        for kk in range(4):
          for c in range(16):
            e = ((rd * 4 + zd) * 4 + zh) * 64 + kk * 16 + c
            src = []
            for j in range(8):
              rh, rw, n = j >> 2, (j >> 1) & 1, j & 1
# ... 5 lines not shown
```

corenet_amd/model/core_net.py:

```python
from __future__ import annotations

import contextlib
import os
import sys
import dataclasses
import math
from typing import Any, Dict, Optional, Tuple

import torch as t
from torch import nn

from corenet_amd import _lib
from corenet_amd.model.engine import Engine, LOSS_KINDS, check_image_hw, on_stream


@dataclasses.dataclass(frozen=True)
class DecoderConfig:
  resolution: Tuple[int, int, int]
  num_output_channels: int
  last_upscale_factor: int = 2
  latent_channels: int = 64
  skip_fraction: float = 0.75


@dataclasses.dataclass(frozen=True)
class CoreNetConfig:
  decoder: DecoderConfig

  def to_dict(self) -> Dict[str, Any]:
    return {"decoder": dataclasses.asdict(self.decoder)}

  @classmethod
  def from_dict(cls, d) -> "CoreNetConfig":
    dd = dict(d["decoder"])
    dd["resolution"] = tuple(dd["resolution"])
    return cls(decoder=DecoderConfig(**dd))


_LIVE_GRAPHS = []


def _release_graphs():
  while _LIVE_GRAPHS:
    try:
      _LIVE_GRAPHS.pop().reset()
    except Exception:
      pass
  try:
    Engine.drain_orphans()
  except Exception:
    pass


import atexit
atexit.register(_release_graphs)


class _Tree(nn.Module):

  def add(self, path, tensor: t.Tensor, kind: str):
    head, *rest = path
    if rest:
      if head not in self._modules:
        self.add_module(head, _Tree())
      self._modules[head].add(rest, tensor, kind)
    elif kind == "param":
      self.register_parameter(head, nn.Parameter(tensor))
    else:
      self.register_buffer(head, tensor)


class _CoreNetFn(t.autograd.Function):

  @staticmethod
  def forward(ctx, model, image, v2s, offset, *params):
    plan = model.engine.plan(image.shape[0], image.shape[2:])
    logits = plan.forward(image, v2s, offset, training=model.training)
    ctx.model, ctx.plan, ctx.generation = model, plan, plan.generation
    return logits.clone()

  @staticmethod
  def backward(ctx, glogits):
    model, plan = ctx.model, ctx.plan
    with model._on_device():
      return _CoreNetFn._backward(ctx, model, plan, glogits)

  @staticmethod
  def _backward(ctx, model, plan, glogits):
    if plan.generation != ctx.generation:
      raise RuntimeError("corenet_amd.CoreNet: backward() of a forward pass whose saved activations were "
                         "overwritten by a later forward with the same batch size; run backward before the "
                         "next forward (gradient accumulation: forward, backward, forward, backward)")
    plan.glogits.copy_(glogits)
    plan.backward(plan.glogits)
    store = model.engine.store
    grads = store.grads.clone()
    return (None, None, None, None) + tuple(store.view_of(grads, k) for k in model._param_keys)


class CoreNet(nn.Module):

  def __init__(self, config, device: Optional[str] = None, backend=None, decoder_math: Optional[str] = None):
    super().__init__()
    self.config = config
    dc = config.decoder
    if device is None:
      device = f"cuda:{t.cuda.current_device()}" if t.cuda.is_available() else "cuda"
    self.engine = Engine(dc.num_output_channels, resolution=tuple(dc.resolution),
                         latent_channels=dc.latent_channels, skip_fraction=dc.skip_fraction,
                         last_upscale_factor=dc.last_upscale_factor, device=device, backend=backend,
                         decoder_math=decoder_math)
    self._packed_version = None
    self._tree_root = _Tree()
    self._param_keys = []
    for key, shape, kind in self.engine.specs:
      self._tree_root.add(key.split("."), self.engine.store.view(key), kind)
      if kind == "param":
        self._param_keys.append(key)
    self.encoder = self._tree_root._modules["encoder"]
    self.decoder = self._tree_root._modules["decoder"]
    del self._tree_root
    self.reset_parameters()
    self.register_load_state_dict_post_hook(lambda m, k: m._mark_dirty())
    self.encoder.register_load_state_dict_post_hook(lambda m, k: self._mark_dirty())

  def _mark_dirty(self):
    self.engine.weights_dirty = True
    self._packed_version = None

  def close(self):
    eng = getattr(self, "engine", None)
    if eng is None:
      return
    live = {id(g) for p in eng.plans.values() for g in list(p.graphs.values()) + [p.eval_graph] if g is not None}
    _LIVE_GRAPHS[:] = [g for g in _LIVE_GRAPHS if id(g) not in live]
    eng.release_graph_resources()

  def __enter__(self):
    return self

  def __exit__(self, *exc):
    self.close()
    return False

  def __del__(self):
    try:
      eng = getattr(self, "engine", None)
      if eng is not None and not sys.is_finalizing():
        live = {id(g) for p in eng.plans.values() for g in list(p.graphs.values()) + [p.eval_graph] if g is not None}
        _LIVE_GRAPHS[:] = [g for g in _LIVE_GRAPHS if id(g) not in live]
        eng.orphan_graph_resources()
    except Exception:
      pass

  def train(self, mode: bool = True):
    self._packed_version = None
    return super().train(mode)

  def _on_device(self):
    d = self.engine.device
    if d.type != "cuda":
      return contextlib.nullcontext()
    stack = contextlib.ExitStack()
    stack.enter_context(t.cuda.device(d))
    stack.enter_context(_lib.pinned_stream())
    return stack

  def reset_parameters(self, seed: int = 0):
    g = t.Generator().manual_seed(seed)
    s = self.engine.store
    with t.no_grad():
      for key, shape, kind in self.engine.specs:
        v = s.view(key)
        if key.endswith("running_var"):
          v.fill_(1.0)
        elif kind != "param":
          v.zero_()
        elif len(shape) >= 2:
          fan_in = shape[1] * int(math.prod(shape[2:])) if len(shape) > 2 else shape[1]
          if key.startswith("encoder."):
            w = t.randn(shape, generator=g) * math.sqrt(2.0 / fan_in)
          else:
            bound = 1.0 / math.sqrt(fan_in)
            w = (t.rand(shape, generator=g) * 2 - 1) * bound
          v.copy_(w)
        elif ".bn." in key or ".b1." in key or ".b2." in key:
          v.fill_(1.0 if key.endswith("weight") else 0.0)
        else:
          v.zero_()
    self._mark_dirty()

  def _apply(self, fn, recurse=True):
    probe = fn(t.zeros(1, device=self.engine.device))
    same = probe.device.type == self.engine.device.type and (
# ... 237 lines not shown
```

corenet_amd/model/engine.py:

```python
from __future__ import annotations

import dataclasses
import os
from typing import Dict, List, Optional, Tuple

import numpy as np
import torch as t

from corenet_amd import _lib
from corenet_amd import views as V
from corenet_amd.backend import Transform
from corenet_amd.model import conv_geometry as G

IMAGE_HW = (256, 256)


def check_image_hw(hw):
  H, W = int(hw[0]), int(hw[1])
  if H < 32 or W < 32 or H % 4 or W % 4 or H * W > 4096 * 4096:
    raise ValueError(f"corenet_amd.CoreNet: image batch of {H}x{W} pixels; this engine takes H and W that are multiples of 4 and >= 32 "
                     f"(256x256 in every shipped config)")
  return H, W
BN_EPS = 1e-3
BN_MOMENTUM = 0.01
# ... 41 lines not shown
  specs.append((d + "stage_1.t1.weight", (latent + 3, 256, 4, 4, 4), "param"))
  specs.append((d + "stage_1.t1.bias", (256,), "param"))
  chans = {2: (256, 128, 3, 3), 3: (128, 64, 5, 7), 4: (64, 32, 5, 7), 5: (32, 16, 5, 7),
           6: (16, num_classes, 5, 7)}
  src_c = {2: 2048, 3: 1024, 4: 512, 5: 256}
  cin = 256
  for st in range(2, 7):
    cmid, cout, k1, k2 = chans[st]
    p = f"{d}stage_{st}."
    bn(p + "b1.", cin)
    conv(p + "c1.", cmid, cin, k1, k1, k1)
    bn(p + "b2.", cmid)
    specs.append((p + "t1.weight", (cmid, cout, k2, k2, k2), "param"))
    specs.append((p + "t1.bias", (cout,), "param"))
    if st in src_c:
      sk = round(cout * skip_fraction)
      conv(f"{d}rt_skip_{st}.compress_channels.", sk, src_c[st] + 3, 1, 1)
      cin = cout + sk
  return specs


class ParamStore:

  def __init__(self, specs, device, dtype=t.float32):
    self.specs = specs
    self.device = device
    self.off: Dict[str, Tuple[int, Tuple[int, ...]]] = {}
    np_, nb, nn = 0, 0, 0
    for key, shape, kind in specs:
      n = int(np.prod(shape)) if len(shape) else 1
      n4 = (n + 3) // 4 * 4
      if kind == "param":
        self.off[key] = (np_, shape); np_ += n4
      elif kind == "buffer":
        self.off[key] = (nb, shape); nb += n4
      else:
        self.off[key] = (nn, shape); nn += 1
    self.kind = {k: kd for k, _, kd in specs}
    self.params = t.zeros(np_, dtype=dtype, device=device)
    self.gslab = t.zeros(np_ + nb, dtype=dtype, device=device)
    self.grads = self.gslab[:np_]
    self.buf_stage = self.gslab[np_:]
    self.buffers = t.zeros(nb, dtype=dtype, device=device)
    self.nbt = t.zeros(nn, dtype=t.int64, device=device)

  def slab(self, key):
    return {"param": self.params, "buffer": self.buffers, "nbt": self.nbt}[self.kind[key]]

  def view(self, key, grad=False) -> t.Tensor:
    o, shape = self.off[key]
    n = int(np.prod(shape)) if len(shape) else 1
    slab = self.grads if grad else self.slab(key)
    return slab[o:o + n].view(shape)

  def offset(self, key) -> int:
    return self.off[key][0]

  def view_of(self, slab: t.Tensor, key) -> t.Tensor:
    o, shape = self.off[key]
    n = int(np.prod(shape)) if len(shape) else 1
    return slab[o:o + n].view(shape)


@dataclasses.dataclass
class BN:
  C: int
  gamma: t.Tensor
  beta: t.Tensor
  rmean: t.Tensor
  rvar: t.Tensor
  nbt: t.Tensor
  dgamma: t.Tensor
  dbeta: t.Tensor
  scale: t.Tensor
  shift: t.Tensor
  saved: t.Tensor


@dataclasses.dataclass
class Conv:
  name: str
  fwd: G.Geom
  dgrad: Optional[G.Geom]
  wf: t.Tensor
  wd: Optional[t.Tensor]
  bias: t.Tensor
  gwf: t.Tensor
  dbias: t.Tensor
  n_ref: int
  wop_f: Optional[t.Tensor] = None
  wop_d: Optional[t.Tensor] = None
  wop_kind: str = ""
  ct_f: Optional[t.Tensor] = None
  ct_d: Optional[t.Tensor] = None
  ct_kind: str = ""


@dataclasses.dataclass(slots=True, eq=False)
class EncBlock:
  prefix: str; stage: str; cin: int; f: Tuple[int, int, int]; stride: int; h: int; w: int
  down: bool
  final: bool
  ya: t.Tensor; yb: t.Tensor; yc: t.Tensor; ys: Optional[t.Tensor]; out: t.Tensor
  gpre: t.Tensor; gyc: t.Tensor; gab: t.Tensor; gyb: t.Tensor; gaa: t.Tensor; gya: t.Tensor
  gys: Optional[t.Tensor]; gin: Optional[t.Tensor]
  xs: Optional[t.Tensor]; gxs: Optional[t.Tensor]
  xs_next: Optional["EncBlock"] = None
  inp: Optional[t.Tensor] = None
  xs_filled: bool = False


@dataclasses.dataclass(slots=True, eq=False)
class DecStage:
  cin: int; cmid: int; cout: int; r: int
  u: t.Tensor; gu: t.Tensor; w: t.Tensor; gw: t.Tensor; gv1: t.Tensor; gv2: t.Tensor

  def __getitem__(self, field: str):
    return getattr(self, field)


class on_stream:
  __slots__ = ("stream", "after", "_torch", "_pin")

  def __init__(self, stream, after=None):
    self.stream, self.after = stream, after
    self._torch, self._pin = t.cuda.stream(stream), _lib.pinned_stream(stream)

  def __enter__(self):
    self._torch.__enter__(); self._pin.__enter__()
    if self.after is not None:
      self.stream.wait_event(self.after)

  def __exit__(self, *exc):
    self._pin.__exit__(*exc); self._torch.__exit__(*exc)


_NO_KW = {}
_ORPHANS = []


class Engine:

  def __init__(self, num_classes: int, resolution=(128, 128, 128), latent_channels: int = 64,
               skip_fraction: float = 0.75, last_upscale_factor: int = 2, device="cuda",
               backend=None, dtype=t.float32, decoder_math: Optional[str] = None):
    if tuple(resolution) != (128, 128, 128) or last_upscale_factor != 2:
      raise ValueError("the CoReNet decoder is only defined for resolution 128^3, "
                       "last_upscale_factor 2 (reconstruction_decoder.py:38-54,93-95)")
    if backend is None:
      from corenet_amd.backend import default_backend
      backend = default_backend()
    self.be = backend
    default_math = "bf16x3" if getattr(backend, "name", "") == "hip" else "fp32"
    self.decoder_math = decoder_math or os.environ.get("CRN_DECODER_MATH", default_math)
    if self.decoder_math not in ("fp32", "bf16x3"):
      raise ValueError(f"decoder_math must be 'fp32' or 'bf16x3', not {self.decoder_math!r}")
    self.encoder_e2d = self.decoder_math == "bf16x3"
    assert dtype == t.float32 or getattr(backend, "name", "") == "emu"
    self.dtype = dtype
    self.device = t.device(device)
    if self.device.type == "cuda" and self.device.index is None:
      self.device = t.device("cuda", t.cuda.current_device() if t.cuda.is_available() else 0)
    self.num_classes = num_classes
    self.latent = latent_channels
    self.resolution = tuple(resolution)
    self.specs = param_specs(num_classes, latent_channels, skip_fraction)
    self.store = ParamStore(self.specs, self.device, dtype)
    self.skip_ch = {2: round(128 * skip_fraction), 3: round(64 * skip_fraction),
                    4: round(32 * skip_fraction), 5: round(16 * skip_fraction)}
    self._build_layers()
    self.plans: Dict[int, "Plan"] = {}
    self.adam_m: Optional[t.Tensor] = None
    self.adam_v: Optional[t.Tensor] = None
    self.adam_t = 0
    self.adam_hyper: Optional[t.Tensor] = None
    self.dgrad_dirty = True
    self.weights_dirty = True
    self.exchange = None
    self._side = False
    self._capture = None
    self._pack_ev = self._dgrad_packed = self._dec_packed = self._enc_late_packed = None
    self._enc_late_pending = False
    self._dec_pack_pending = False
    self._dgrad_pack_pending = False
    self._gpacked_zeroed = False

  def orphan_graph_resources(self):
    graphs = [g for p in self.plans.values() for g in list(p.graphs.values()) + [p.eval_graph] if g is not None]
    for p in self.plans.values():
      p.graphs, p.eval_graph, p.eval_eager = {}, None, 0
    if graphs or self._capture is not None:
      _ORPHANS.append((self.be, graphs, self._capture))
    self._capture = None

  @staticmethod
  def drain_orphans():
    while _ORPHANS:
      be, graphs, stream = _ORPHANS.pop()
      for g in graphs:
        try:
          g.reset()
        except Exception:
          pass
      if stream is not None:
        be.splitk_release(stream)

  def capture_stream(self):
    Engine.drain_orphans()
    if self._capture is None:
      self._capture = t.cuda.Stream(device=self.device)
    self.be.splitk_reserve(self._capture, floats=0)
    return self._capture

  def release_graph_resources(self):
    for p in self.plans.values():
      for g in list(p.graphs.values()) + ([p.eval_graph] if p.eval_graph is not None else []):
        try:
          g.reset()
        except Exception:
          pass
      p.graphs, p.eval_graph, p.eval_eager = {}, None, 0
    if self._capture is not None:
      self.be.splitk_release(self._capture)
      self._capture = None

  def side_stream(self):
    if self._side is False:
      use = self.device.type == "cuda"
      self._side = t.cuda.Stream(device=self.device) if use else None
      if use:
        self._pack_ev, self._dgrad_packed = t.cuda.Event(), t.cuda.Event()
        self._dec_packed, self._enc_late_packed = t.cuda.Event(), t.cuda.Event()
    return self._side

  def _bn(self, prefix: str) -> BN:
    s = self.store
    c = s.off[prefix + "weight"][1][0]
    dev = self.device
    o = self._bn_slab_off[prefix]
    return BN(c, s.view(prefix + "weight"), s.view(prefix + "bias"), s.view(prefix + "running_mean"),
              s.view(prefix + "running_var"), s.view(prefix + "num_batches_tracked"),
              s.view(prefix + "weight", grad=True), s.view(prefix + "bias", grad=True),
              self.bn_scale[o:o + c], self.bn_shift[o:o + c],
              t.zeros(4 * c, device=dev, dtype=self.dtype))

  def _bn_slabs(self):
    s = self.store
    self._bn_slab_off, rows, n = {}, [], 0
    for key, shape, kind in self.specs:
      if not key.endswith("running_mean"):
        continue
      p = key[:-len("running_mean")]
      c = shape[0]
      self._bn_slab_off[p] = n
      ch = np.arange(c)
      rows.append(np.stack([s.offset(p + "weight") + ch, s.offset(p + "bias") + ch, s.offset(p + "running_mean") + ch,
                            s.offset(p + "running_var") + ch, n + ch], 1))
      n += (c + 3) // 4 * 4
    self.bn_scale = t.zeros(n, device=self.device, dtype=self.dtype)
    self.bn_shift = t.zeros(n, device=self.device, dtype=self.dtype)
    self.bn_eval_table = t.as_tensor(np.concatenate(rows).astype(np.int32), device=self.device)

  def bn_eval_affine(self):
    self.be.bn_eval_affine(self.store.params, self.store.buffers, self.bn_eval_table, BN_EPS, self.bn_scale,
                           self.bn_shift)

  def _build_layers(self):
    s = self.store
    self.convs: Dict[str, Conv] = {}
    self.bns: Dict[str, BN] = {}
    self._bn_slabs()
    reg: List[Tuple[str, G.Geom, Optional[G.Geom], int, int]] = []

    def add(name, fwd, dgrad, repeat=1):
      nref = s.off[name + "bias"][1][0]
      reg.append((name, fwd, dgrad, repeat, nref))

    for key, shape, kind in self.specs:
      if kind != "param" or not key.endswith("weight") or len(shape) < 4:
        if key.endswith("running_mean"):
          p = key[:-len("running_mean")]
          self.bns[p] = self._bn(p)
        continue
      name = key[:-len("weight")]
      if name == "encoder.stage1.conv.":
        add(name, G.stem_fwd(shape, 3), None)
      elif name == "decoder.stage_1.t1.":
        add(name, G.convt_1to4_fwd(shape), G.convt_1to4_dgrad(shape), repeat=64)
      elif ".t1." in name:
        p = 1 if shape[2] == 3 else 3
        add(name, G.convt_fwd(shape, p), G.convt_dgrad(shape, p), repeat=8)
      else:
        p = shape[-1] // 2
        add(name, G.conv_fwd(shape, p), G.conv_dgrad(shape, p))
    idx_parts, sizes = [], []
    for name, fwd, dgrad, repeat, nref in reg:
      wo, bo = s.offset(name + "weight"), s.offset(name + "bias")
      def shift(ix, o):
        return np.where(ix >= 0, ix.astype(np.int64) + o, -1)
      parts = [shift(fwd.index, wo), shift(G.bias_index(nref, repeat, fwd.npad, parity_major=(repeat == 8)), bo)]
      if dgrad is not None:
        alias = (len(dgrad.index) == int(np.prod(s.off[name + "weight"][1]))
                 and np.array_equal(dgrad.index, np.arange(len(dgrad.index))))
        parts.append(np.zeros(0, np.int64) if alias else shift(dgrad.index, wo))
      idx_parts.append(parts)
    flat_len = sum(len(p) for parts in idx_parts for p in parts)
    assert max(int(p.max()) for parts in idx_parts for p in parts if len(p)) < 2 ** 31
    self.packed = t.zeros(flat_len, dtype=self.dtype, device=self.device)
    gsize = sum(len(parts[0]) for parts in idx_parts)
    self.gpacked = t.zeros(gsize, dtype=self.dtype, device=self.device)
    pack_parts, pack_is_bwd, pack_names, unpack_parts = [], [], [], []
    po, go = 0, 0
    for (name, fwd, dgrad, repeat, nref), parts in zip(reg, idx_parts):
      pack_parts.append((po, parts[0], fwd.npad, 0)); po += len(parts[0]); pack_is_bwd.append(False); pack_names.append(name)
      pack_parts.append((po, parts[1], len(parts[1]), 0)); po += len(parts[1]); pack_is_bwd.append(False); pack_names.append(name)
      if dgrad is not None and len(parts[2]):
        pack_parts.append((po, parts[2], dgrad.npad, dgrad.taps if dgrad.taps > 1 else 0)); po += len(parts[2])
        pack_is_bwd.append(True); pack_names.append(name)
      unpack_parts.append((go, parts[0], fwd.npad, 0)); go += len(parts[0])
    dev = self._tiles_dev
    self.pack_tiles = dev([pp for pp, bwd in zip(pack_parts, pack_is_bwd) if not bwd])
    sel = lambda pred: [pp for pp, bwd, nm in zip(pack_parts, pack_is_bwd, pack_names) if not bwd and pred(nm)]
    early = lambda nm: nm.startswith("encoder.stage1") or nm.startswith("encoder.stage2")
    self.pack_tiles_enc = dev(sel(lambda nm: nm.startswith("encoder.")))
    self.pack_tiles_enc_early = dev(sel(early))
    self.pack_tiles_enc_late = dev(sel(lambda nm: nm.startswith("encoder.") and not early(nm)))
    self.pack_tiles_dec = dev(sel(lambda nm: not nm.startswith("encoder.")))
    self.pack_tiles_bwd = dev([pp for pp, bwd in zip(pack_parts, pack_is_bwd) if bwd])
    self.unpack_tiles = dev(unpack_parts)
    los = [min(o for k, (o, _) in s.off.items() if s.kind[k] == "param" and k.startswith(lb))
           for lb in GRAD_BUCKET_LABELS[:-1]] + [0]
    self.grad_buckets: List[Tuple[str, int, int]] = []
    self._bucket_tiles = []
    hi = s.params.numel()
    for lb, lo in zip(GRAD_BUCKET_LABELS, los):
      assert lo < hi
      self.grad_buckets.append((lb, lo, hi))
      sel = [up for (name, *_), up in zip(reg, unpack_parts) if lo <= s.offset(name + "weight") < hi]
      self._bucket_tiles.append(sel)
      hi = lo
    self._bucket_dev = None
    po, go = 0, 0
    for (name, fwd, dgrad, repeat, nref), parts in zip(reg, idx_parts):
      nwf, nb = len(parts[0]), len(parts[1])
      wf = self.packed[po:po + nwf]; po += nwf
      bias = self.packed[po:po + nb]; po += nb
      wd = None
      if dgrad is not None:
        if len(parts[2]):
          wd = self.packed[po:po + len(parts[2])]; po += len(parts[2])
        else:
          wd = s.view(name + "weight").view(-1)
      gwf = self.gpacked[go:go + nwf]; go += nwf
      self.convs[name] = Conv(name, fwd, dgrad, wf, wd, bias, gwf,
                              s.view(name + "bias", grad=True), nref)
    self._build_operands(reg, idx_parts)

  def _build_ct_images(self):
    self.ct_tables = {}
    name = "decoder.stage_6.t1."
    if (self.decoder_math != "bf16x3" or self.device.type != "cuda"
        or name not in self.convs or not hasattr(self.be, "convt_par_fwd")):
      return
    shape = tuple(self.store.off[name + "weight"][1])
    if shape[0] != 16 or shape[1] > 16 or tuple(shape[2:]) != (7, 7, 7) or tuple(self.resolution) != (128, 128, 128):
      return
    if shape[1] == 2:
      kind_, tabs = "res", (G.convt_res_fwd_table, G.convt_res_dgrad_table)
    elif shape[1] >= CT_PAR_MIN:
      kind_, tabs = "par", (G.convt_par_fwd_table, G.convt_par_dgrad_table)
    else:
      return
    self.convs[name].ct_kind = kind_
    wofs = self.store.offset(name + "weight")
    for kind, fn, field in (("dec", tabs[0], "ct_f"), ("bwd", tabs[1], "ct_d")):
      tab, nbytes = fn(shape, wofs)
      img = t.zeros(nbytes, dtype=t.uint8, device=self.device)
      setattr(self.convs[name], field, img)
      self.ct_tables[kind] = (t.as_tensor(tab, device=self.device), img)

  def _build_operands(self, reg, idx_parts):
    self.wop = None
    self.op_tables = {}
    self._build_ct_images()
    if self.decoder_math != "bf16x3":
      return
    groups = {"enc_early": [], "enc_late": [], "dec": [], "bwd": []}
    slices = []
    po, eo = 0, 0
    for (name, fwd, dgrad, repeat, nref), parts in zip(reg, idx_parts):
      src_f = po; po += len(parts[0]) + len(parts[1])
      src_d = po
      if dgrad is not None:
        po += len(parts[2])
      if (name, "fwd") in BF16X3_LAUNCHES:
        groups["dec"].append((src_f, eo, fwd, True))
        slices.append((name, "wop_f", eo, G.slab_entries(fwd))); eo += G.slab_entries(fwd)
        groups["bwd"].append((src_d, eo, dgrad, True))
        slices.append((name, "wop_d", eo, G.slab_entries(dgrad))); eo += G.slab_entries(dgrad)
        self.convs[name].wop_kind = "slab"
        continue
      if not self.encoder_e2d or not name.startswith("encoder.") or name.startswith("encoder.stage1"):
        continue
      self.convs[name].wop_kind = "e2d"
      if fwd.window != (1, 3, 3):
        continue
      if G.operand_eligible(fwd) and name[len("encoder.stage")] in "45":
        groups["enc_early" if name.startswith("encoder.stage2") else "enc_late"].append((src_f, eo, fwd))
        slices.append((name, "wop_f", eo, G.operand_entries(fwd))); eo += G.operand_entries(fwd)
      if dgrad is not None and len(parts[2]) and G.operand_eligible(dgrad):
        groups["bwd"].append((src_d, eo, dgrad))
        slices.append((name, "wop_d", eo, G.operand_entries(dgrad))); eo += G.operand_entries(dgrad)
    if not eo:
      return
    self.wop = t.zeros(eo * 32, dtype=t.uint8, device=self.device)
    for name, field, e0, n in slices:
      setattr(self.convs[name], field, self.wop[e0 * 32:(e0 + n) * 32])
    for k, layers in groups.items():
      if layers:
        desc, blocks = G.operand_table(layers)
        self.op_tables[k] = (t.as_tensor(desc, device=self.device), blocks)

  def _operands(self, *groups):
    for k in groups:
      if k in self.op_tables:
        self.be.bf3_operands(self.packed, self.op_tables[k], self.wop)
      if k in self.ct_tables:
        self.be.bf3_gather_image(self.store.params, *self.ct_tables[k])

  def _tiles_dev(self, parts):
    mats, rest = G.mat_index(parts)
    tl = G.tile_index(rest)
    return (t.as_tensor(tl[0], device=self.device), t.as_tensor(tl[1].view(np.int64), device=self.device),
            t.as_tensor(tl[2] if tl[2].size else np.zeros(1, np.int32), device=self.device),
            t.as_tensor(mats, device=self.device))

  def bucket_unpack_tiles(self, i: int):
    if self._bucket_dev is None:
      self._bucket_dev = [self._tiles_dev(sel) for sel in self._bucket_tiles]
    return self._bucket_dev[i]

  @property
  def weights_dirty(self) -> bool:
    return self._weights_dirty

  @weights_dirty.setter
  def weights_dirty(self, v: bool):
    self._weights_dirty = v
    if v:
      self.dgrad_dirty = True

  def pack_weights(self, part: str = "all"):
    tiles = {"all": self.pack_tiles, "enc": self.pack_tiles_enc, "dec": self.pack_tiles_dec,
             "enc_early": self.pack_tiles_enc_early, "enc_late": self.pack_tiles_enc_late}[part]
    self.be.copy_tiles(self.store.params, self.packed, tiles)
    self._operands(*{"all": ("enc_early", "enc_late", "dec"), "enc": ("enc_early", "enc_late"), "dec": ("dec",),
                     "enc_early": ("enc_early",), "enc_late": ("enc_late",)}[part])
    if part in ("all", "dec"):
      self._weights_dirty = False

  def pack_dgrad_weights(self):
    self.be.copy_tiles(self.store.params, self.packed, self.pack_tiles_bwd)
    self._operands("bwd")
    self.dgrad_dirty = False

  def plan(self, batch: int, hw=IMAGE_HW) -> "Plan":
    hw = (int(hw[0]), int(hw[1]))
    key = batch if hw == IMAGE_HW else (batch, hw[0], hw[1])
    p = self.plans.get(key)
    if p is None:
      p = Plan(self, batch, hw)
      self.plans[key] = p
    return p

  def adam_step(self, lr: float, eps: float, betas=(0.9, 0.999), grad_scale: float = 1.0):
    if self.adam_m is None:
      self.adam_m = t.zeros_like(self.store.params)
      self.adam_v = t.zeros_like(self.store.params)
    self.adam_t += 1
    self.be.adam_step(self.store.params, self.store.grads, self.adam_m, self.adam_v,
                      self.store.params.numel(), lr, betas[0], betas[1], eps, grad_scale, self.adam_t)
    self.weights_dirty = True

  def adam_step_graphable(self, lr: float, eps: float, betas=(0.9, 0.999), grad_scale: float = 1.0, launch: bool = True):
    if self.adam_m is None:
      self.adam_m = t.zeros_like(self.store.params)
      self.adam_v = t.zeros_like(self.store.params)
    if self.adam_hyper is None:
      self.adam_hyper = t.zeros(8, dtype=t.float32, device=self.device)
    self.adam_t += 1
    self.be.adam_set_hyper(self.adam_hyper, lr, betas[0], betas[1], eps, grad_scale, self.adam_t)
    if launch:
      self.adam_update_from_hyper()

  def adam_bucket_hook(self):
    def hook(gslice: t.Tensor):
      lo, n = gslice.storage_offset(), gslice.numel()
      self.be.adam_step_hyper(self.store.params[lo:lo + n], gslice, self.adam_m[lo:lo + n], self.adam_v[lo:lo + n], n,
                              self.adam_hyper)
    return hook

  def adam_update_from_hyper(self):
    self.be.adam_step_hyper(self.store.params, self.store.grads, self.adam_m, self.adam_v,
                            self.store.params.numel(), self.adam_hyper)
    self.weights_dirty = True


def _no_exchange(grads: t.Tensor):
  """Bucket hook of a step without a gradient exchange."""


class Plan:

  def __init__(self, eng: Engine, B: int, hw=IMAGE_HW):
    self.eng, self.B = eng, B
    H, W = check_image_hw(hw)
    self.hw = (H, W)
    self.stem_hw = (H // 2, W // 2)
    parts = int(eng.be.lib.crn_stem_conv_parts(B, H, W)) if hasattr(eng.be, "stem_conv_fwd") else 0
    self.stem_fast = 0 < parts <= 4096
    self.dec_stats_fused = hasattr(eng.be, "conv_fwd_stats")
    self.pool_hw = (H // 4, W // 4)
    self.be = eng.be
    self.generation = 0
    self.graphs = {}
    self.eager_steps = 0
    self.eval_graph = None
    self.eval_eager = 0
    self._views = {}
    dev = eng.device
    self.dev = dev
    f = lambda *shape: t.zeros(*shape, dtype=eng.dtype, device=dev)
    self.in_image = t.zeros(B, 3, H, W, dtype=t.uint8, device=dev)
    self.in_v2s = f(B, 4, 4)
    self.in_off = f(B, 3)
    self.img = f(B, 3, H, W)
    self.y1 = f(B, 64, *self.stem_hw)
    self.gy1 = f(B, 64, *self.stem_hw); self.gy1b = f(B, 64, *self.stem_hw)
    self.p1 = f(B, 64, *self.pool_hw)
    self.p1_arg = t.zeros(B, 64, *self.pool_hw, dtype=t.int32, device=dev)
    self.blocks = []
    cin, (hi, wi) = 64, self.pool_hw
    stage_hw = {}
    for name, blocks, filt, stride in ENC_STAGES:
      for bl in blocks:
        st = stride if bl == "a" else 1
        ho, wo = (hi + st - 1) // st, (wi + st - 1) // st
        z = lambda c: f(B, c, ho, wo)
        s2 = st == 2
        blk = EncBlock(prefix=f"encoder.{name}.{bl}.", stage=name, cin=cin, f=filt, stride=st, h=ho, w=wo, down=(bl == "a"),
                       final=(bl == blocks[-1]), ya=z(filt[0]), yb=z(filt[1]), yc=z(filt[2]), ys=z(filt[2]) if bl == "a" else None,
                       out=z(filt[2]), gpre=z(filt[2]), gyc=z(filt[2]), gab=z(filt[1]), gyb=z(filt[1]), gaa=z(filt[0]), gya=z(filt[0]),
                       gys=z(filt[2]) if bl == "a" else None, gin=f(B, cin, hi, wi) if bl == "a" else None,
                       xs=z(cin) if s2 else None, gxs=z(cin) if s2 else None)
        if s2 and self.blocks:
          self.blocks[-1].xs_next = blk
        self.blocks.append(blk)
        cin, hi, wi = filt[2], ho, wo
      stage_hw[name] = (hi, wi)
    self.stage_hw = stage_hw
    self.feat = {"stage2": f(B, 256 + 3, *stage_hw["stage2"]), "stage3": f(B, 512 + 3, *stage_hw["stage3"]),
                 "stage4": f(B, 1024 + 3, *stage_hw["stage4"]), "stage5": f(B, 2048 + 3, *stage_hw["stage5"])}
    self.gfeat = {k: t.zeros_like(v) for k, v in self.feat.items()}
    self.avg = f(B, 2048); self.gavg = f(B, 2048)
    L = eng.latent
    self.z0 = f(B, L + 3); self.gz0 = f(B, L + 3); self.gv0 = f(B, L + 3)
    C = eng.num_classes
    sk = eng.skip_ch
    self.dec = {}
    for k, (ci, cm, co, r) in {2: (256, 256, 128, 4), 3: (128 + sk[2], 128, 64, 8), 4: (64 + sk[3], 64, 32, 16),
                               5: (32 + sk[4], 32, 16, 32), 6: (16 + sk[5], 16, C, 64)}.items():
      self.dec[k] = DecStage(ci, cm, co, r, u=f(B, ci, r, r, r), gu=f(B, ci, r, r, r), w=f(B, cm, r, r, r), gw=f(B, cm, r, r, r),
                             gv1=f(B, ci, r, r, r), gv2=f(B, cm, r, r, r))
    self.logits = f(B, C, 128, 128, 128)
    self.glogits = f(B, C, 128, 128, 128)
    self.skip_src = {2: "stage5", 3: "stage4", 4: "stage3", 5: "stage2"}
    self.skip_hw = {k: stage_hw[self.skip_src[k]] for k in self.skip_src}
    self.smap = {k: f(B, self.skip_hw[k][0], self.skip_hw[k][1], sk[k]) for k in sk}
    self.ray_idx = ({k: t.zeros(B, (2 * self.dec[k].r) ** 3, dtype=t.int16, device=dev) for k in sk}
                    if hasattr(self.be, "ray_sample_fwd_idx") and max(h * w for h, w in self.skip_hw.values()) < 65535 else None)
    gs_n = {k: B * sk[k] * self.skip_hw[k][0] * self.skip_hw[k][1] for k in sk}
    self.gsmap_slab = f(sum(gs_n.values()))
    self.gsmap, o = {}, 0
    for k in sk:
      self.gsmap[k] = self.gsmap_slab[o:o + gs_n[k]].view(B, sk[k], *self.skip_hw[k]); o += gs_n[k]
    self.layer_mats = f(4, B, 16)
    self._layer_scale_list = [128.0 / (2 * self.dec[k].r) for k in (2, 3, 4, 5)]
    self.layer_scales = t.tensor([[128.0 / (2 * self.dec[k].r)] * 3 + [1.0] for k in (2, 3, 4, 5)],
                                 dtype=eng.dtype, device=dev).reshape(4, 1, 1, 4)
    self.offset = f(B, 3)
    self.loss = f(1)
    self.gt = t.zeros(B, 128, 128, 128, dtype=t.int32, device=dev)
    self.side = eng.side_stream()
    use_side = self.side is not None
    self._side_ev, self._side_i = [], 0
    self._side_done = t.cuda.Event() if use_side else None
    self._ximg_ev = t.cuda.Event() if use_side else None
    self._ct_ximg = self._ct_ximg_buf = None
    self._handed_over = False
    self._g_compact = None
    self._wg_pending = []
    self._skip_ev = {k: (t.cuda.Event(), t.cuda.Event()) for k in (2, 3, 4, 5)} if use_side else None
    self._skip_bwd_ev = {k: t.cuda.Event() for k in (2, 3, 4, 5)} if use_side else None
    self._skip_bwd_done = t.cuda.Event() if use_side else None
    self._skip_async_live = False

  def _cached(self, key, fn):
    v = self._views.get(key)
    if v is None:
      v = fn()
      self._views[key] = v
    return v

  def vw(self, x: t.Tensor) -> V.View:
    return self._cached(("v", x.data_ptr(), tuple(x.shape), tuple(x.stride())), lambda: V.view_of(x))

  def s2d(self, x: t.Tensor, c1: int, r) -> V.View:
    pm = tuple(r) == (2, 2, 2)
    return self._cached(("s2d", x.data_ptr(), tuple(x.shape), tuple(x.stride()), c1, r),
                        lambda: V.space_to_depth_view(self.vw(x).channels(0, c1), r, parity_major=pm))

  def flat(self, x: t.Tensor) -> V.View:
    return self._cached(("flat", x.data_ptr(), tuple(x.shape)), lambda: V.flat_channel_view(self.vw(x)))

  probes = None

  def _probe(self, name: str, fn):
    if self.probes is None or name not in self.probes:
      return fn()
    a, b = t.cuda.Event(enable_timing=True), t.cuda.Event(enable_timing=True)
    a.record(); r = fn(); b.record()
    self.probes[name].append((a, b))
    return r

  @property
  def overlap(self) -> bool:
    return self.side is not None and self.trace is None

  def _on_side(self, after=None):
    return on_stream(self.side, after)

  def _next_handover_event(self):
    if self._side_i == len(self._side_ev):
      self._side_ev.append(t.cuda.Event())
    ev = self._side_ev[self._side_i]; self._side_i += 1
    ev.record()
    return ev

  def _stats(self, bn: BN, x: t.Tensor, S: int, sB: int, pre_relu: bool, training: bool):
    if not training:
      return
    with _lib.roctx_range("bn_stats C%d S%d" % (bn.C, S)):
      self.be.bn_stats(x, self.B, bn.C, S, sB, pre_relu, bn.gamma, bn.beta, bn.rmean, bn.rvar, bn.nbt,
                       BN_EPS, BN_MOMENTUM, True, bn.scale, bn.shift, bn.saved)

  def _bn_finalize(self, b: BN, parts: int, count: int):
    self.be.bn_finalize(parts, b.C, count, b.gamma, b.beta, b.rmean, b.rvar, b.nbt, BN_EPS, BN_MOMENTUM, b.scale, b.shift, b.saved)

  def _bn_bwd(self, b: BN, x: t.Tensor, dy: t.Tensor, dx: t.Tensor, S: int, pre_relu: bool, post_relu: bool, bias_of: Optional[Conv] = None):
    n = b.C * S
    self.be.bn_bwd(x, n, dy, n, self.B, b.C, S, pre_relu, post_relu, b.gamma, b.scale, b.shift, b.saved, dx, n, b.dgamma, b.dbeta,
                   dsum=None if bias_of is None else bias_of.dbias, ndsum=0 if bias_of is None else bias_of.n_ref)

  trace = None

  def _timed(self, label, fn):
    if _lib.ROCTX:
      with _lib.roctx_range(label):
        return fn()
    if self.trace is None:
      return fn()
    a, b = t.cuda.Event(enable_timing=True), t.cuda.Event(enable_timing=True)
    a.record(); r = fn(); b.record()
    self.trace.append((label, a, b))
    return r

  def _math(self, cv: Conv, direction: str) -> str:
    if cv.wop_kind == "e2d" and (direction == "fwd" and cv.wop_f is not None or
                                 direction == "dgrad" and cv.wop_d is not None):
      return "e2d"
    return "bf16x3" if self.eng.decoder_math == "bf16x3" and (cv.name, direction) in BF16X3_LAUNCHES else "fp32"

  conv_positions = None

  @staticmethod
  def _e2d_shape_ok(v: V.View, window) -> bool:
    S = v.D * v.H * v.W
    if S % 4:
      return False
    if tuple(window) == (1, 3, 3):
      tw = 16 if v.W % 16 == 0 else 8
      return v.D == 1 and v.W % tw == 0 and v.H % (64 // tw) == 0
    return S % 64 == 0

  @staticmethod
  def _wg2d_shape_ok(v: V.View, window) -> bool:
    return (v.D * v.H * v.W) % 32 == 0 and (tuple(window) == (1, 1, 1) or v.W % 8 == 0)

  def _conv(self, cv: Conv, x: V.View, tr, y: V.View, accumulate=False):
    g = cv.fwd
    if self.conv_positions is not None:
      self.conv_positions[cv.name] = y.D * y.H * y.W
    if cv.wop_f is not None and cv.wop_kind == "e2d" and self._e2d_shape_ok(y, g.window):
      self._timed("fwd   " + cv.name, lambda: self.be.conv2d_bf3(
          x, tr, cv.wop_f, g.npad, cv.bias, 0, y, g.window, g.pad_lo, accumulate))
      return
    self._timed("fwd   " + cv.name, lambda: self.be.conv_fwd(
        x, tr, cv.wf, g.npad, cv.bias, 0, y, g.window, g.pad_lo, 0, accumulate, boxes=(g.n_boxes, g.c_boxes),
        math=self._math(cv, "fwd"), wslab=cv.wop_f if cv.wop_kind == "slab" else None))

  def _dgrad(self, cv: Conv, dy: V.View, dx: V.View, accumulate=False):
    g = cv.dgrad
    if cv.wop_d is not None and cv.wop_kind == "e2d" and self._e2d_shape_ok(dx, g.window):
      self._timed("dgrad " + cv.name, lambda: self.be.conv2d_bf3(
          dy, None, cv.wop_d, g.npad, None, 0, dx, g.window, g.pad_lo, accumulate))
      return
    self._timed("dgrad " + cv.name, lambda: self.be.conv_fwd(
        dy, None, cv.wd, g.npad, None, 0, dx, g.window, g.pad_lo, 0, accumulate, boxes=(g.n_boxes, g.c_boxes),
        math=self._math(cv, "dgrad"), wslab=cv.wop_d if cv.wop_kind == "slab" else None))

  def _dgrad_bn_bwd(self, cv: Conv, dy: V.View, g: t.Tensor, x: t.Tensor, Cn: int, S: int, b, dx: t.Tensor, cprev: Conv) -> bool:
    be = self.be
    gvw = self.vw(g)
    fusable = (hasattr(be, "conv_dgrad_bn_bwd") and cv.wop_kind == "slab" and cv.wop_d is not None
               and self._math(cv, "dgrad") == "bf16x3")
    if not fusable:
      be.splitk_defer()
      self._dgrad(cv, dy, gvw)
      return False
    gd = cv.dgrad
    be.splitk_defer()
    return self._timed("dgrad " + cv.name, lambda: be.conv_dgrad_bn_bwd(
        dy, cv.wop_d, gd.npad, gvw, g, gd.window, gd.pad_lo, (gd.n_boxes, gd.c_boxes), x, Cn * S, self.B, Cn, S, True, b.gamma,
        b.scale, b.shift, b.saved, dx, Cn * S, b.dgamma, b.dbeta, dsum=cprev.dbias, ndsum=cprev.n_ref))

  def _wgrad_math(self, cv: Conv, dy: V.View) -> str:
    g = cv.fwd
    math = self._math(cv, "wgrad")
    if self.stem_fast and cv.name == "encoder.stage1.conv.":
      math = "stem"
    if (self.eng.encoder_e2d and g.window in ((1, 1, 1), (1, 3, 3)) and self._wg2d_shape_ok(dy, g.window)
        and (cv.name.startswith("encoder.stage") and not cv.name.startswith("encoder.stage1")
             or cv.name.startswith("decoder.rt_skip"))):
      math = "bf16x3_2d"
    if cv.ct_kind == "par" and math == "bf16x3":
      math = "ct_par"
    return math

  def _launch_wgrad(self, cv: Conv, x: V.View, tr, dy: V.View, math: str, kw: dict):
    g = cv.fwd
    with _lib.roctx_range("wgrad " + cv.name):
      self.be.conv_wgrad(x, tr, dy, cv.gwf, g.npad, g.window, g.pad_lo, False, boxes=(g.n_boxes, g.c_boxes), math=math, **kw)

  def _wgrad(self, cv: Conv, x: V.View, tr, dy: V.View, here: bool = False):
    math = self._wgrad_math(cv, dy)
    kw = self._ximg_kw(math)
    if here:
      return self._launch_wgrad(cv, x, tr, dy, math, kw)
    if not self.overlap:
      return self._timed("wgrad " + cv.name, lambda: self._launch_wgrad(cv, x, tr, dy, math, kw))
    if cv.name.startswith("encoder."):
      self._wg_pending.append((cv, x, tr, dy, math, kw))
      return
    if self._handed_over:
      self._handed_over = False
      self._side_i = max(self._side_i, 1)
      ev = None
    else:
      ev = self._next_handover_event()
    with self._on_side(after=ev):
      self._launch_wgrad(cv, x, tr, dy, math, kw)

  def _ximg_kw(self, math: str) -> dict:
    if math != "ct_par" or self._ct_ximg is None:
      return _NO_KW
    img, self._ct_ximg = self._ct_ximg, None
    return {"ximg": img}

  def _flush_wgrads(self, then=None):
    if not self._wg_pending and then is None:
      return
    with self._on_side(after=self._next_handover_event()):
      for args in self._wg_pending:
        self._launch_wgrad(*args)
      if then is not None:
        then()
    self._wg_pending = []

  def _join_side(self):
    self._flush_wgrads()
    if self._side_i:
      self._side_done.record(self.side)
      t.cuda.current_stream().wait_event(self._side_done)
      self._side_i = 0

  def _bias_grad(self, cv: Conv, dy: t.Tensor, S: int, sB: int):
    self.be.bias_grad(dy, self.B, cv.n_ref, S, sB, cv.dbias)

  def forward(self, image_u8: t.Tensor, v2s: t.Tensor, offset: t.Tensor, training: bool) -> t.Tensor:
    self._skip_async_live = bool(training and self.overlap)
    if self._skip_async_live:
      self._decoder_inputs(v2s, offset)
# ... 407 lines not shown
```

include/corenet_hip.h:

```cpp
#ifndef CORENET_HIP_H_
#define CORENET_HIP_H_

#include <stddef.h>
#include <stdint.h>

#ifdef __cplusplus
extern "C" {
#endif

#define CRN_OK 0
#define CRN_EINVAL (-1)
#define CRN_ENOMEM (-2)
#define CRN_ENOCONV (-3)

typedef void* crnStream;

typedef struct {
  float* base;
  int32_t B, C, D, H, W;
  int64_t sB, sC;
  const int32_t* chan_off;
  int32_t sD, sH, sW;
} crnView;

typedef struct {
  const float* scale;
  const float* shift;
  int32_t pre_relu, post_relu;
} crnInTransform;

typedef struct {
  int32_t n_groups, c_groups;
  int8_t n_box[8][6];
  int8_t c_box[8][6];
} crnTapBoxes;

int crn_conv_fwd(const crnView* x, const crnInTransform* tr, const float* w, int Npad,
                 const float* bias, int bias_sB, const crnView* y,
                 int kd, int kh, int kw, int pd, int ph, int pw,
                 int splits, int accumulate ,
                 const crnTapBoxes* boxes , crnStream stream);

#define CRN_PLAN_DENSE_COLS 1
#define CRN_PLAN_DENSE_ROWS 2
#define CRN_PLAN_DENSE_WGRAD 3
#define CRN_PLAN_POINTWISE 4
#define CRN_PLAN_GENERIC 5
typedef struct {
  int32_t path;
  int32_t msub, nsub;
  int32_t xstage, dystage;
  int32_t forced;
  int32_t cc;
  int32_t td, th, tw;
  int32_t mw;
  int32_t splits;
  int32_t chunks;
  int32_t vec_store;
  int32_t balanced;
  int32_t lds_bytes, lds_budget;
} crnConvPlan;
int crn_conv_fwd_plan(const crnView* x, const crnInTransform* tr, const float* w, int Npad,
                      const float* bias, int bias_sB, const crnView* y,
                      int kd, int kh, int kw, int pd, int ph, int pw,
                      int splits, int accumulate, const crnTapBoxes* boxes, crnConvPlan* out);

int crn_conv_fwd_bf3(const crnView* x, const crnInTransform* tr, const float* w, int Npad,
                     const float* bias, int bias_sB, const crnView* y,
                     int kd, int kh, int kw, int pd, int ph, int pw,
                     int accumulate, const crnTapBoxes* boxes , crnStream stream);

int crn_conv_fwd_bf3_slabs(const crnView* x, const crnInTransform* tr, const void* wslab, int Npad,
                           const float* bias, int bias_sB, const crnView* y,
                           int kd, int kh, int kw, int pd, int ph, int pw,
                           int accumulate, const crnTapBoxes* boxes , crnStream stream);

typedef struct crnBnBwdFuse {
  const float* x;
  int64_t sB_x;
  const float* saved;
  int pre_relu;
  double* ws; size_t ws_bytes;
  float* dsum; int ndsum;
  int nparts;
} crnBnBwdFuse;
int crn_conv_fwd_bf3_slabs_bnbwd(const crnView* x, const crnInTransform* tr, const void* wslab, int Npad,
                                 const float* bias, int bias_sB, const crnView* y,
                                 int kd, int kh, int kw, int pd, int ph, int pw,
                                 int accumulate, const crnTapBoxes* boxes , crnBnBwdFuse* fuse,
                                 crnStream stream);

int crn_conv_fwd_bf3_slabs_stats(const crnView* x, const crnInTransform* tr, const void* wslab, int Npad,
                                 const float* bias, int bias_sB, const crnView* y,
                                 int kd, int kh, int kw, int pd, int ph, int pw,
                                 int accumulate, const crnTapBoxes* boxes , int pre_relu,
                                 double* ws, size_t ws_bytes, int* nparts, crnStream stream);

int crn_splitk_defer(int on);
int crn_splitk_reserve(int64_t floats, crnStream stream);
int crn_splitk_release(crnStream stream);

int crn_conv_wgrad(const crnView* x, const crnInTransform* tr, const crnView* dy,
                   float* dw, int Npad, int kd, int kh, int kw, int pd, int ph, int pw,
                   int zero_first, const crnTapBoxes* boxes ,
                   crnStream stream);

int crn_conv_wgrad_plan(const crnView* x, const crnInTransform* tr, const crnView* dy,
                        float* dw, int Npad, int kd, int kh, int kw, int pd, int ph, int pw,
                        int zero_first, const crnTapBoxes* boxes, crnConvPlan* out);

int crn_conv_wgrad_bf3(const crnView* x, const crnInTransform* tr, const crnView* dy,
                       float* dw, int Npad, int kd, int kh, int kw, int pd, int ph, int pw,
                       int zero_first, crnStream stream);
int crn_conv_wgrad_bf3_boxes(const crnView* x, const crnInTransform* tr, const crnView* dy, float* dw, int Npad,
                             int kd, int kh, int kw, int pd, int ph, int pw, int zero_first,
                             const crnTapBoxes* boxes , crnStream stream);

#define CRN_BF3_PLAIN 0
#define CRN_BF3_HALF 1
#define CRN_BF3_WS 2
typedef struct {
  int32_t kind;
  int32_t nsub;
  int32_t xmode;
  int32_t ng;
  int32_t slabs;
  int32_t td, th, tw;
  int32_t splits;
  int32_t chunks;
  int32_t per_split;
  int32_t vec_store, mode;
  int32_t rowskip, half_last;
  int32_t lead;
  int32_t n_groups, c_groups;
  int32_t nparts;
  int32_t dmode, tpw, twt;
  int32_t pipe, inherit, boxskip;
  int32_t lds_bytes;
} crnBf3Plan;
int crn_conv_fwd_bf3_plan(const crnView* x, const crnInTransform* tr, const float* w, const void* wslab, int Npad,
                          const float* bias, int bias_sB, const crnView* y,
                          int kd, int kh, int kw, int pd, int ph, int pw,
                          int accumulate, const crnTapBoxes* boxes, const crnBnBwdFuse* fuse, crnBf3Plan* out);
int crn_conv_wgrad_bf3_plan(const crnView* x, const crnInTransform* tr, const crnView* dy, float* dw, int Npad,
                            int kd, int kh, int kw, int pd, int ph, int pw, int zero_first,
                            const crnTapBoxes* boxes, crnBf3Plan* out);

int crn_bf3_operands(const float* packed, const int64_t* desc, int nlayers, int64_t total_blocks, void* out,
                     crnStream stream);
int crn_conv2d_bf3(const crnView* x, const crnInTransform* tr, const void* wop, int Npad, const float* bias,
                   int bias_sB, const crnView* y, int kh, int kw, int ph, int pw, int accumulate, crnStream stream);

int crn_conv_wgrad_1x1_bf3(const crnView* x, const crnInTransform* tr, const crnView* dy, float* dw, int Npad,
                           int zero_first, crnStream stream);
int crn_conv_wgrad_2d_bf3(const crnView* x, const crnInTransform* tr, const crnView* dy, float* dw, int Npad,
                          int kh, int kw, int ph, int pw, int zero_first, crnStream stream);

int crn_copy_tiles_f32(const float* src, float* dst, const int32_t* desc ,
                       const uint64_t* mask , const int32_t* explicit_idx, int64_t ntiles,
                       int reverse, crnStream s);
int crn_copy_mats_f32(const float* src, float* dst, const int32_t* desc , int64_t nblocks,
                      int reverse, crnStream s);
int crn_gather_f32(const float* src, const int32_t* idx, float* dst, int64_t n, crnStream s);
int crn_scatter_f32(const float* src, const int32_t* idx, float* dst, int64_t n,
                    int accumulate, crnStream s);
int crn_bias_grad(const float* dy, int B, int C, int64_t S, int64_t sB, float* db,
                  int accumulate, double* workspace ,
                  size_t workspace_bytes, crnStream s);

int crn_batch_renorm_stats(const float* x, int B, int C, int64_t S, int64_t sB, int pre_relu,
                           const float* gamma, const float* beta,
                           float* running_mean, float* running_var,
                           const int64_t* num_batches_tracked ,
                           float eps, float momentum, int training,
                           float* scale, float* shift, float* saved ,
                           double* workspace, size_t workspace_bytes, crnStream s);
size_t crn_batch_renorm_workspace_bytes(int C);
int crn_batch_renorm_stats_tail(const float* x, int B, int C, int64_t S, int64_t sB,
                                const float* gamma, const float* beta, float* running_mean, float* running_var,
                                const int64_t* num_batches_tracked, float eps, float momentum, int training,
                                float* scale, float* shift, float* saved, double* workspace, size_t workspace_bytes,
                                const float* r, const float* rscale, const float* rshift, int64_t sB_r,
                                float* y_pre, int64_t sB_pre, float* y, int64_t sB_y, int relu,
                                float* y2, int W, crnStream s);

int crn_batch_renorm_eval_affine(const float* params, const float* buffers, const int32_t* table,
                                 int n, float eps, float* scale, float* shift, crnStream s);

int crn_batch_renorm_bwd(const float* x, int64_t sB_x, const float* dy, int64_t sB_dy,
                         int B, int C, int64_t S, int pre_relu, int post_relu,
                         const float* gamma, const float* scale, const float* shift,
                         const float* saved, float* dx, int64_t sB_dx,
                         float* dgamma, float* dbeta, int accumulate,
                         float* dsum, int ndsum,
                         double* workspace, size_t workspace_bytes, crnStream s);

int crn_batch_renorm_bwd_apply(const float* x, int64_t sB_x, const float* dy, int64_t sB_dy,
                               int B, int C, int64_t S, int pre_relu,
                               const float* gamma, const float* scale, const float* shift,
                               const float* saved, float* dx, int64_t sB_dx,
                               float* dgamma, float* dbeta, int accumulate,
                               float* dsum, int ndsum,
                               double* workspace, size_t workspace_bytes, int nparts, crnStream s);

int crn_batch_renorm_bwd_head(const float* x, int64_t sB_x, float* dy, int64_t sB_dy,
                              const float* g, int64_t sB_g, const float* act, int64_t sB_act,
                              const float* g2 , int64_t sB_g2,
                              int B, int C, int64_t S, const float* gamma, const float* scale, const float* shift,
                              const float* saved, float* dx, int64_t sB_dx, float* dgamma, float* dbeta,
                              int accumulate, float* dsum, int ndsum,
                              double* workspace, size_t workspace_bytes, const float* g_compact, int W, crnStream s);

int crn_affine_add_relu(const float* x, const float* scale, const float* shift,
                        const float* r, const float* rscale, const float* rshift,
                        int B, int C, int64_t S, int64_t sB_x, int64_t sB_r,
                        float* y_pre, int64_t sB_pre, float* y, int64_t sB_y,
                        int relu, crnStream s);

int crn_relu_bwd_add(const float* dy, const float* y_pre, const float* dy2,
                     int B, int C, int64_t S, int64_t sB_dy, int64_t sB_pre, int64_t sB_dy2,
                     float* dx, int64_t sB_dx, crnStream s);

size_t crn_stem_conv_parts(int B, int H, int W);
int crn_stem_conv_fwd(const float* img, int B, int H, int W, const float* w_packed, const float* bias,
                      float* y, double* stats_ws , size_t ws_bytes, crnStream s);
int crn_stem_conv_wgrad(const float* img, int B, int H, int W, const float* dy, float* dw_packed, crnStream s);
int crn_batch_renorm_finalize(const double* ws, int nparts, int C, double count,
                              const float* gamma, const float* beta, float* running_mean, float* running_var,
                              const int64_t* nbt, float eps, float momentum,
                              float* scale, float* shift, float* saved, crnStream s);

int crn_preprocess_caffe(const uint8_t* img, int B, int H, int W, float* out, crnStream s);
// ... 177 lines not shown
```

Measured before the change: 1.195 billion.

## Build bf16x3 operands and pointwise weights directly from parameter storage

Result: no change. 1.199 billion, median of 2 (+0.4%).

```diff
diff --git a/corenet_amd/_lib.py b/corenet_amd/_lib.py
--- a/corenet_amd/_lib.py
+++ b/corenet_amd/_lib.py
@@ -88,6 +88,9 @@
     "crn_conv_wgrad": [C.POINTER(CrnView), C.POINTER(CrnInTransform), C.POINTER(CrnView), vp, i32,
                        i32, i32, i32, i32, i32, i32, i32, vp, vp],
     "crn_bf3_operands": [vp, vp, i32, i64, vp, vp],
+    "crn_bf3_operands_slab": [vp, vp, i32, i64, vp, i32, vp, vp],
+    "crn_conv_fwd_nk": [C.POINTER(CrnView), C.POINTER(CrnInTransform), vp, vp, i32, C.POINTER(CrnView), i32, vp],
+    "crn_conv_fwd_nk_plan": [C.POINTER(CrnView), C.POINTER(CrnInTransform), vp, C.POINTER(CrnView)],
     "crn_bf3_gather_image": [vp, vp, i32, vp, vp],
     "crn_convt_s2k7_fwd_bf3": [vp, i64, i32, i32, i32, i32, C.POINTER(CrnInTransform), vp, vp, vp, i64, i64, i32, vp],
     "crn_convt_s2k7_dgrad_bf3": [vp, i64, i64, i32, i32, i32, i32, i32, vp, vp, i64, i32, vp],
diff --git a/corenet_amd/backend.py b/corenet_amd/backend.py
--- a/corenet_amd/backend.py
+++ b/corenet_amd/backend.py
@@ -91,6 +91,18 @@
                           pad_lo[0], pad_lo[1], pad_lo[2], splits, int(accumulate), _ctapboxes(boxes),
                           _lib.stream())
 
+  def conv_fwd_nk(self, x: View, tr: Optional[Transform], w: t.Tensor, bias: Optional[t.Tensor], bias_sB: int, y: View,
+                  accumulate: bool = False):
+    self.lib.crn_conv_fwd_nk(C.byref(_cview(x)), _ctr(tr), ptr(w), ptr(bias), bias_sB, C.byref(_cview(y)), int(accumulate),
+                             _lib.stream())
+
+  def conv_fwd_nk_ok(self, x: View, tr: Optional[Transform], w: t.Tensor, y: View) -> bool:
+    try:
+      self.lib.crn_conv_fwd_nk_plan(C.byref(_cview(x)), _ctr(tr), ptr(w), C.byref(_cview(y)))
+    except _lib.HipError:
+      return False
+    return True
+
   @staticmethod
   def _plan_dict(p) -> dict:
     d = {n: int(getattr(p, n)) for n, _ in p._fields_}
@@ -171,6 +183,10 @@
   def bf3_operands(self, packed: t.Tensor, table, out: t.Tensor):
     desc, blocks = table
     self.lib.crn_bf3_operands(ptr(packed), ptr(desc), desc.shape[0], blocks, ptr(out), _lib.stream())
+
+  def bf3_operands_slab(self, params: t.Tensor, table, out: t.Tensor):
+    desc, blocks, tab, lds = table
+    self.lib.crn_bf3_operands_slab(ptr(params), ptr(desc), desc.shape[0], blocks, ptr(tab), lds, ptr(out), _lib.stream())
 
   def bf3_gather_image(self, src: t.Tensor, table: t.Tensor, out: t.Tensor, host_table=None):
     self.lib.crn_bf3_gather_image(ptr(src), ptr(table), table.shape[0], ptr(out), _lib.stream())
diff --git a/corenet_amd/csrc/conv_e2d.hip b/corenet_amd/csrc/conv_e2d.hip
--- a/corenet_amd/csrc/conv_e2d.hip
+++ b/corenet_amd/csrc/conv_e2d.hip
@@ -76,6 +76,98 @@
   bf16x8* dst = reinterpret_cast<bf16x8*>(out + (d[1] + e) * 32);
   dst[0] = h;
   dst[1] = l;
+}
+
+constexpr int kOpSlabFields = 13;
+
+__device__ __forceinline__ long long bf3_entry_index(int T, int Npad, int KHW, int chunk, int t, int n) {
+  if (KHW > 0) {
+    const int kd = T / KHW, TP = (KHW + 3) & ~3, zd = t / KHW, tp = t - zd * KHW;
+    return (((long long)chunk * kd + zd) * TP + tp) * Npad + n;
+  }
+  const int ntn = Npad >> 4;
+  return (((long long)(chunk >> 2) * T + t) * ntn + (n >> 4)) * 64 + (chunk & 3) * 16 + (n & 15);
+}
+
+__global__ __launch_bounds__(256) void bf3_operands_slab_kernel(const float* slab, const long long* desc, int nlayers,
+                                                                const int* table, char* out) {
+  extern __shared__ float tile[];
+  int lo = 0, hi = nlayers - 1;
+  while (lo < hi) {
+    const int mid = (lo + hi + 1) >> 1;
+    if (desc[mid * kOpSlabFields + 5] <= (long long)blockIdx.x) lo = mid; else hi = mid - 1;
+  }
+  const long long* d = desc + lo * kOpSlabFields;
+  const int Cin = (int)d[2], T = (int)d[3], Npad = (int)d[4], KHW = (int)d[6], kind = (int)d[11];
+  const long long sc = d[7];
+  const int wg = (int)((long long)blockIdx.x - d[5]), tid = threadIdx.x;
+  bf16x8* dst = reinterpret_cast<bf16x8*>(out + d[1] * 32);
+  if (kind == 2) {
+    const int kd = T / KHW, TP = (KHW + 3) & ~3;
+    const long long entries = (long long)((Cin + 7) >> 3) * kd * TP * Npad;
+    long long e = (long long)wg * 256 + tid;
+    if ((256 % TP) == 0 && (Npad % (256 / TP)) == 0) {
+      const int ncol = 256 / TP, gpr = Npad / ncol;
+      const int tp = tid % TP, nl = tid / TP;
+      const long long row = wg / gpr;
+      e = (row * TP + tp) * Npad + (long long)(wg - row * gpr) * ncol + nl;
+    }
+    if (e >= entries) return;
+    const int chunk = (int)(e / ((long long)kd * TP * Npad));
+    const int* tab = table + d[0];
+    const int b = tab[e];
+    float v[8];
+#pragma unroll
+    for (int j = 0; j < 8; ++j) {
+      long long ix = -1;
+      if (b >= 0) ix = chunk * 8 + j < Cin ? b + j * sc : -1;
+      else if (b < -1) ix = tab[entries + (long long)(-2 - b) * 8 + j];
+      v[j] = ix >= 0 ? slab[ix] : 0.f;
+    }
+    bf16x8 h, l;
+    split8(v, h, l);
+    dst[e * 2] = h;
+    dst[e * 2 + 1] = l;
+    return;
+  }
+  const long long st = d[8], sn = d[9];
+  const int N = (int)d[10], NB = (int)d[12];
+  const int ngrp = (Npad + NB - 1) / NB;
+  const int chunk = wg / ngrp, n0 = (wg - chunk * ngrp) * NB, c0 = chunk * 8;
+  const int run = kind == 0 ? 8 * T : NB * T, P = run | 1, rows = kind == 0 ? NB : 8;
+  const int rmax = kind == 0 ? min(8, Cin - c0) * T : max(0, min(NB, N - n0)) * T;
+  const int rowmax = kind == 0 ? max(0, min(NB, N - n0)) : min(8, Cin - c0);
+  const long long base = kind == 0 ? d[0] + (long long)n0 * sn + c0 * sc
+                                   : d[0] + (long long)c0 * sc + (long long)n0 * sn + (st < 0 ? -(T - 1) : 0);
+  const long long rstride = kind == 0 ? sn : sc;
+  for (int r = tid; r < run; r += 256) {
+    float v[16];
+#pragma unroll
+    for (int q = 0; q < 16; ++q) v[q] = (q < rowmax && r < rmax) ? slab[base + q * rstride + r] : 0.f;
+#pragma unroll
+    for (int q = 0; q < 16; ++q)
+      if (q < rows) tile[q * P + r] = v[q];
+  }
+  __syncthreads();
+  const int TP = KHW > 0 ? (KHW + 3) & ~3 : 1, kd = KHW > 0 ? T / KHW : T;
+  const int nent = kd * TP * NB, lgNB = 31 - __clz(NB);
+  for (int i = tid; i < nent; i += 256) {
+    const int nl = i & (NB - 1), r = i >> lgNB, zd = r / TP, tp = r - zd * TP;
+    const int n = n0 + nl;
+    if (n >= Npad) continue;
+    const bool real = KHW == 0 || tp < KHW;
+    const int t = KHW > 0 ? zd * KHW + tp : zd;
+    const float* src = kind == 0 ? tile + nl * P + t : tile + nl * T + (st < 0 ? T - 1 - t : t);
+    const int js = kind == 0 ? T : P;
+    float v[8];
+#pragma unroll
+    for (int j = 0; j < 8; ++j) v[j] = real ? src[j * js] : 0.f;
+    bf16x8 h, l;
+    split8(v, h, l);
+    const long long e = KHW > 0 ? (((long long)chunk * kd + zd) * TP + tp) * Npad + n : bf3_entry_index(T, Npad, 0, chunk, t, n);
+    dst[e * 2] = h;
+    dst[e * 2 + 1] = l;
+  }
 }
 
 constexpr unsigned kOOB = 0x80000000u;
@@ -636,6 +728,18 @@
   if (!packed || !desc || !out || nlayers < 1 || total_blocks < 1 || total_blocks > 0x7fffffff) return CRN_EINVAL;
   hipLaunchKernelGGL(bf3_operands_kernel, dim3((unsigned)total_blocks), dim3(256), 0, (hipStream_t)stream, packed,
                      reinterpret_cast<const long long*>(desc), nlayers, reinterpret_cast<char*>(out));
+  CRN_CHECK_LAUNCH();
+  return CRN_OK;
+}
+
+extern "C" int crn_bf3_operands_slab(const float* slab, const int64_t* desc, int nlayers, int64_t total_blocks,
+                                     const int32_t* table, int lds_bytes, void* out, crnStream stream) {
+  CRN_ENTRY(stream);
+  if (!slab || !desc || !out || nlayers < 1 || total_blocks < 1 || total_blocks > 0x7fffffff || lds_bytes < 0 ||
+      lds_bytes > 65536)
+    return CRN_EINVAL;
+  hipLaunchKernelGGL(bf3_operands_slab_kernel, dim3((unsigned)total_blocks), dim3(256), (size_t)lds_bytes, (hipStream_t)stream,
+                     slab, reinterpret_cast<const long long*>(desc), nlayers, table, reinterpret_cast<char*>(out));
   CRN_CHECK_LAUNCH();
   return CRN_OK;
 }
diff --git a/corenet_amd/csrc/conv_igemm.hip b/corenet_amd/csrc/conv_igemm.hip
--- a/corenet_amd/csrc/conv_igemm.hip
+++ b/corenet_amd/csrc/conv_igemm.hip
@@ -20,12 +20,14 @@
 
 constexpr int kPwBN = 32;
 constexpr int kPwTab = 2048;
-template <int NS>
-__global__ __launch_bounds__(256) void pointwise_fwd_kernel(PwGeom g) {
+template <int NS, bool NK>
+__device__ __forceinline__ void pointwise_fwd_body(const PwGeom& g) {
   constexpr int BM = 64, BN = NS * 16, KC = 64, SA = BM + 16, SB = BN + 16;
+  constexpr int SBK = KC + 2;
   constexpr int NRA = KC / 16;
+  static_assert(!NK || NS == 2, "the [n][k] staging roles below cover 32 rows x 16 float4 with two loads per thread");
   __shared__ __attribute__((aligned(16))) float ldsA[KC * SA];
-  __shared__ __attribute__((aligned(16))) float ldsB[KC * SB];
+  __shared__ __attribute__((aligned(16))) float ldsB[NK ? BN * SBK : KC * SB];
   crn_kernargs_now(g.x, g.y, g.w, g.bias, g.tr.scale, g.tr.shift, g.tr.pre_relu, g.tr.post_relu, g.B, g.C, g.N, g.Npad,
                    g.S, g.xsB, g.ysB, g.ysC, g.ysP, g.bias_sB, g.mode, g.splits, g.cps);
   const long long t_entry = (long long)__builtin_amdgcn_s_memtime();
@@ -43,8 +45,9 @@
   const int ka = tid >> 4, ca = (tid & 15) * 4;
   constexpr int BQ = BN / 4, BROWS = 256 / BQ, NRB = KC / BROWS;
   const int kb = tid / BQ, cb = (tid % BQ) * 4;
+  const int nlb = (tid >> 4) * 2 + ((tid & 15) >> 3), kqb = (tid & 7) * 4;
   const bool a_ok = (m0 + ca) < g.S;
-  const bool b_ok = (n0 + cb) < g.Npad;
+  const bool b_ok = NK ? (n0 + nlb) < g.N : (n0 + cb) < g.Npad;
   extern __shared__ float pw_tables[];
   const bool has_tr = g.tr.scale != nullptr;
   float* tsc = pw_tables; float* tsh = pw_tables + g.cps;
@@ -62,8 +65,9 @@
     }
 #pragma unroll
     for (int q = 0; q < NRB; ++q) {
-      const int c_b = c0 + kb + q * BROWS;
-      const unsigned off = (b_ok && c_b < cend) ? (unsigned)(c_b * g.Npad + n0 + cb) * 4u : kOOBo;
+      const int c_b = NK ? c0 + kqb + q * 32 : c0 + kb + q * BROWS;
+      const unsigned off = !(b_ok && c_b < cend) ? kOOBo
+                           : NK ? (unsigned)((n0 + nlb) * g.C + c_b) * 4u : (unsigned)(c_b * g.Npad + n0 + cb) * 4u;
       crnk::crn_bload4(pb_[q], wrs, off);
     }
   };
@@ -102,18 +106,26 @@
 #pragma unroll
     for (int q = 0; q < NRA; ++q) *reinterpret_cast<f32x4*>(ldsA + (ka + q * 16) * SA + ca) = xform(pa_[q], c0 + ka + q * 16);
 #pragma unroll
-    for (int q = 0; q < NRB; ++q) *reinterpret_cast<f32x4*>(ldsB + (kb + q * BROWS) * SB + cb) = pb_[q];
+    for (int q = 0; q < NRB; ++q) {
+      if constexpr (NK) {
+        float2* d2 = reinterpret_cast<float2*>(ldsB + nlb * SBK + kqb + q * 32);
+        d2[0] = make_float2(pb_[q][0], pb_[q][1]);
+        d2[1] = make_float2(pb_[q][2], pb_[q][3]);
+      } else {
+        *reinterpret_cast<f32x4*>(ldsB + (kb + q * BROWS) * SB + cb) = pb_[q];
+      }
+    }
     __syncthreads();
     mark();
     issue(c0 + 2 * KC, pa_, pb_);
     const float* pa = ldsA + kk * SA + wave * 16 + i16;
-    const float* pb = ldsB + kk * SB + i16;
+    const float* pb = NK ? ldsB + i16 * SBK + kk : ldsB + kk * SB + i16;
 #pragma unroll
     for (int ks = 0; ks < KC / 4; ++ks) {
       const float a = pa[ks * 4 * SA];
       float bv[NS];
 #pragma unroll
-      for (int ns = 0; ns < NS; ++ns) bv[ns] = pb[ks * 4 * SB + ns * 16];
+      for (int ns = 0; ns < NS; ++ns) bv[ns] = NK ? pb[ks * 4 + ns * 16 * SBK] : pb[ks * 4 * SB + ns * 16];
 #pragma unroll
       for (int ns = 0; ns < NS; ++ns) acc[ns] = __builtin_amdgcn_mfma_f32_16x16x4f32(a, bv[ns], acc[ns], 0, 0, 0);
     }
@@ -154,6 +166,10 @@
     g.stamps[30] = (long long)__builtin_amdgcn_s_memrealtime() - r_entry;
   }
 }
+template <int NS>
+__global__ __launch_bounds__(256) void pointwise_fwd_kernel(PwGeom g) { pointwise_fwd_body<NS, false>(g); }
+template <int NS>
+__global__ __launch_bounds__(256) void pointwise_fwd_nk_kernel(PwGeom g) { pointwise_fwd_body<NS, true>(g); }
 
 constexpr int kDenseB = 8;
 __global__ __launch_bounds__(256) void dense_cols_kernel(const float* x, int64_t xsB, int64_t xsC, crnInTransform tr,
@@ -475,6 +491,42 @@
   return CRN_OK;
 }
 #endif
+static int pw_launch(const crnView* x, const crnInTransform* tr, const float* w, int Npad, const float* bias, int bias_sB,
+                     const crnView* y, int accumulate, const FwdSel& sel, bool armed, bool nk, hipStream_t st) {
+  const int64_t Sx = (int64_t)x->D * x->H * x->W;
+  PwGeom p{};
+  p.x = x->base; p.y = y->base; p.w = w; p.bias = bias;
+  p.tr = tr ? *tr : crnInTransform{nullptr, nullptr, 0, 0};
+  p.B = x->B; p.C = x->C; p.N = y->C; p.Npad = Npad; p.S = (int)Sx;
+  p.xsB = x->sB; p.ysB = y->sB; p.bias_sB = bias_sB; p.mode = accumulate ? 1 : 0;
+  p.ysC = y->sC; p.ysP = y->sW;
+  p.splits = 1; p.cps = sel.pw_cps_whole;
+  const int64_t ytot = (int64_t)y->B * y->C * Sx;
+  float* scratch = nullptr;
+  if (sel.pw_splits > 1 && (scratch = crn_splitk_scratch((size_t)sel.pw_splits * ytot, st)) != nullptr) {
+    p.splits = sel.pw_splits; p.cps = sel.pw_cps;
+    p.y = scratch; p.ysB = (int64_t)y->C * Sx; p.ysC = Sx; p.ysP = 1; p.mode = 0;
+  }
+#ifdef CRN_TOOLS
+  static const bool want_stamps = getenv("CRN_PW_STAMPS") != nullptr;
+#else
+  constexpr bool want_stamps = false;
+#endif
+  static long long* pw_stamps = nullptr;
+  if (want_stamps) {
+    if (!pw_stamps) CRN_HIP(hipMalloc(&pw_stamps, 32 * sizeof(long long)));
+    CRN_HIP(hipMemsetAsync(pw_stamps, 0, 32 * sizeof(long long), st));
+    p.stamps = pw_stamps;
+    g_pw_stamps = pw_stamps;
+  }
+  dim3 grid((unsigned)crn_cdiv(Sx, 64), (unsigned)crn_cdiv(y->C, kPwBN), (unsigned)(x->B * p.splits));
+  const size_t tab_bytes = p.tr.scale ? (size_t)2 * p.cps * sizeof(float) : 0;
+  if (nk) hipLaunchKernelGGL(pointwise_fwd_nk_kernel<kPwBN / 16>, grid, dim3(256), tab_bytes, st, p);
+  else hipLaunchKernelGGL(pointwise_fwd_kernel<kPwBN / 16>, grid, dim3(256), tab_bytes, st, p);
+  CRN_CHECK_LAUNCH();
+  return p.splits > 1 ? crn_splitk_finish(*y, scratch, p.splits, accumulate, armed, st) : CRN_OK;
+}
+
 extern "C" int crn_conv_fwd(const crnView* x, const crnInTransform* tr, const float* w, int Npad,
                             const float* bias, int bias_sB, const crnView* y,
                             int kd, int kh, int kw, int pd, int ph, int pw,
@@ -507,38 +559,7 @@
     CRN_CHECK_LAUNCH();
     return CRN_OK;
   }
-  if (sel.path == CRN_PLAN_POINTWISE) {
-    PwGeom p{};
-    p.x = x->base; p.y = y->base; p.w = w; p.bias = bias;
-    p.tr = tr ? *tr : crnInTransform{nullptr, nullptr, 0, 0};
-    p.B = x->B; p.C = x->C; p.N = y->C; p.Npad = Npad; p.S = (int)Sx;
-    p.xsB = x->sB; p.ysB = y->sB; p.bias_sB = bias_sB; p.mode = accumulate ? 1 : 0;
-    p.ysC = y->sC; p.ysP = y->sW;
-    p.splits = 1; p.cps = sel.pw_cps_whole;
-    const int64_t ytot = (int64_t)y->B * y->C * Sx;
-    float* scratch = nullptr;
-    if (sel.pw_splits > 1 && (scratch = crn_splitk_scratch((size_t)sel.pw_splits * ytot, st)) != nullptr) {
-      p.splits = sel.pw_splits; p.cps = sel.pw_cps;
-      p.y = scratch; p.ysB = (int64_t)y->C * Sx; p.ysC = Sx; p.ysP = 1; p.mode = 0;
-    }
-#ifdef CRN_TOOLS
-    static const bool want_stamps = getenv("CRN_PW_STAMPS") != nullptr;
-#else
-    constexpr bool want_stamps = false;
-#endif
-    static long long* pw_stamps = nullptr;
-    if (want_stamps) {
-      if (!pw_stamps) CRN_HIP(hipMalloc(&pw_stamps, 32 * sizeof(long long)));
-      CRN_HIP(hipMemsetAsync(pw_stamps, 0, 32 * sizeof(long long), st));
-      p.stamps = pw_stamps;
-      g_pw_stamps = pw_stamps;
-    }
-    dim3 grid((unsigned)crn_cdiv(Sx, 64), (unsigned)crn_cdiv(y->C, kPwBN), (unsigned)(x->B * p.splits));
-    const size_t tab_bytes = p.tr.scale ? (size_t)2 * p.cps * sizeof(float) : 0;
-    hipLaunchKernelGGL(pointwise_fwd_kernel<kPwBN / 16>, grid, dim3(256), tab_bytes, st, p);
-    CRN_CHECK_LAUNCH();
-    return p.splits > 1 ? crn_splitk_finish(*y, scratch, p.splits, accumulate, armed, st) : CRN_OK;
-  }
+  if (sel.path == CRN_PLAN_POINTWISE) return pw_launch(x, tr, w, Npad, bias, bias_sB, y, accumulate, sel, armed, false, st);
   const FwdCfg& best = sel.cfg;
   const int xvec = sel.xvec, lead = sel.lead;
   splits = sel.splits;
@@ -591,6 +612,29 @@
 #undef CRN_FWD_CASE
   if (rc == CRN_OK && g.mode == 3) rc = crn_splitk_finish(yreal, scratch, splits, accumulate, armed, st);
   return rc;
+}
+
+static int nk_select(const crnView* x, const crnInTransform* tr, const float* w, const crnView* y, FwdSel* sel) {
+  if (!x || !y || !w || x->B != y->B || (x->C & 3) || y->C < 1) return CRN_EINVAL;
+  const int npad = (y->C + 15) & ~15;
+  const int rcs = fwd_select(x, tr, w, npad, y, 1, 1, 1, 0, 0, 0, 0, sel);
+  if (rcs != CRN_OK) return rcs;
+  return sel->path == CRN_PLAN_POINTWISE ? CRN_OK : CRN_EINVAL;
+}
+extern "C" int crn_conv_fwd_nk_plan(const crnView* x, const crnInTransform* tr, const float* w, const crnView* y) {
+  FwdSel sel;
+  return nk_select(x, tr, w, y, &sel);
+}
+extern "C" int crn_conv_fwd_nk(const crnView* x, const crnInTransform* tr, const float* w, const float* bias, int bias_sB,
+                               const crnView* y, int accumulate, crnStream stream) {
+  FwdSel sel;
+  const int rcn = nk_select(x, tr, w, y, &sel);
+  if (rcn != CRN_OK) return rcn;
+  hipStream_t st = (hipStream_t)stream;
+  int rcf;
+  const bool armed = crn_splitk_begin(st, &rcf);
+  if (rcf != CRN_OK) return rcf;
+  return pw_launch(x, tr, w, (y->C + 15) & ~15, bias, bias_sB, y, accumulate, sel, armed, true, st);
 }
 
 namespace {
diff --git a/corenet_amd/model/conv_geometry.py b/corenet_amd/model/conv_geometry.py
--- a/corenet_amd/model/conv_geometry.py
+++ b/corenet_amd/model/conv_geometry.py
@@ -300,6 +300,77 @@
   return np.asarray(rows, dtype=np.int64).reshape(-1, 7), blocks
 
 
+OP_SLAB_LDS = 40960
+
+
+def _affine_map(g: Geom):
+  idx3 = np.asarray(g.index, np.int64).reshape(g.cin, g.taps, g.npad)
+  v = idx3 >= 0
+  N = int(v[0, 0].sum())
+  if N == 0 or not v[:, :, :N].all() or v[:, :, N:].any():
+    return None
+  base = int(idx3[0, 0, 0])
+  sc = int(idx3[1, 0, 0]) - base if g.cin > 1 else 0
+  st = int(idx3[0, 1, 0]) - base if g.taps > 1 else 0
+  sn = int(idx3[0, 0, 1]) - base if N > 1 else 0
+  pred = (base + np.arange(g.cin)[:, None, None] * sc + np.arange(g.taps)[None, :, None] * st + np.arange(N)[None, None, :] * sn)
+  return (base, sc, st, sn, N) if (pred == idx3[:, :, :N]).all() else None
+
+
+def _entry_table(g: Geom, wofs: int):
+  khw, kd = g.window[1] * g.window[2], g.window[0]
+  tp, chunks = (khw + 3) // 4 * 4, (g.cin + 7) // 8
+  full = np.full((chunks * 8, kd, tp, g.npad), -1, np.int64)
+  full[:g.cin, :, :khw] = np.asarray(g.index, np.int64).reshape(g.cin, kd, khw, g.npad)
+  idx8 = full.reshape(chunks, 8, kd, tp, g.npad).transpose(0, 2, 3, 4, 1).reshape(-1, 8)
+  live = np.arange(chunks * 8).reshape(chunks, 1, 1, 1, 8) < g.cin
+  live = np.broadcast_to(live, (chunks, kd, tp, g.npad, 8)).reshape(-1, 8)
+  both = (idx8[:, 0] >= 0) & (idx8[:, 1] >= 0)
+  diffs = (idx8[:, 1] - idx8[:, 0])[both]
+  sc = int(np.bincount(diffs - diffs.min()).argmax() + diffs.min()) if diffs.size else 0
+  empty = (idx8 < 0).all(1)
+  pred = idx8[:, :1] + np.arange(8)[None, :] * sc
+  affine = ~empty & (idx8[:, 0] >= 0) & np.where(live, idx8 == pred, idx8 < 0).all(1)
+  explicit = ~empty & ~affine
+  vals = np.where(empty, -1, idx8[:, 0] + wofs)
+  vals[explicit] = -2 - np.arange(int(explicit.sum()))
+  rows = idx8[explicit]
+  rows = np.where(rows >= 0, rows + wofs, -1)
+  return sc, np.concatenate([vals, rows.reshape(-1)])
+
+
+def operand_slab_table(layers):
+  rows, blocks, tabs, tab_len, lds = [], 0, [], 0, 0
+  for layer in layers:
+    wofs, dst, g = layer[:3]
+    slab = len(layer) > 3 and layer[3]
+    khw = g.window[1] * g.window[2] if slab else 0
+    am = _affine_map(g)
+    T = g.taps
+    kind = None if am is None else (0 if am[1] == T and am[2] == (1 if T > 1 else 0) else
+                                    1 if am[3] == T and am[2] == (-1 if T > 1 else 0) else None)
+    if kind is not None:
+      base, sc, st, sn, N = am
+      tile = lambda nb: (nb * ((8 * T) | 1) if kind == 0 else 8 * ((nb * T) | 1)) * 4
+      nb = 16
+      while nb > 1 and tile(nb) > OP_SLAB_LDS:
+        nb //= 2
+      assert tile(nb) <= 65536
+      lds = max(lds, tile(nb))
+      rows.append((wofs + base, dst, g.cin, T, g.npad, blocks, khw, sc, st, sn, N, kind, nb))
+      chunks = (g.cin + 7) // 8 if slab else g.cin // 8
+      blocks += chunks * ((g.npad + nb - 1) // nb)
+    else:
+      assert slab, "operand blocks of the encoder engine: plain convolutions only"
+      sc, tab = _entry_table(g, wofs)
+      assert np.abs(tab).max(initial=0) < 2 ** 31
+      rows.append((tab_len, dst, g.cin, g.taps, g.npad, blocks, khw, sc, 0, 0, g.nout, 2, 0))
+      tabs.append(tab.astype(np.int32)); tab_len += len(tab)
+      blocks += (slab_entries(g) + 255) // 256
+  table = np.concatenate(tabs) if tabs else None
+  return np.asarray(rows, dtype=np.int64).reshape(-1, 13), blocks, table, lds
+
+
 def _ct_table(rows_of_step):
   tab, off16 = [], 0
   for rows, entry in rows_of_step:
diff --git a/corenet_amd/model/core_net.py b/corenet_amd/model/core_net.py
--- a/corenet_amd/model/core_net.py
+++ b/corenet_amd/model/core_net.py
@@ -100,7 +100,8 @@
 
 class CoreNet(nn.Module):
 
-  def __init__(self, config, device: Optional[str] = None, backend=None, decoder_math: Optional[str] = None):
+  def __init__(self, config, device: Optional[str] = None, backend=None, decoder_math: Optional[str] = None,
+               full_pack: bool = False):
     super().__init__()
     self.config = config
     dc = config.decoder
@@ -109,7 +110,7 @@
     self.engine = Engine(dc.num_output_channels, resolution=tuple(dc.resolution),
                          latent_channels=dc.latent_channels, skip_fraction=dc.skip_fraction,
                          last_upscale_factor=dc.last_upscale_factor, device=device, backend=backend,
-                         decoder_math=decoder_math)
+                         decoder_math=decoder_math, full_pack=full_pack)
     self._packed_version = None
     self._tree_root = _Tree()
     self._param_keys = []
diff --git a/corenet_amd/model/engine.py b/corenet_amd/model/engine.py
--- a/corenet_amd/model/engine.py
+++ b/corenet_amd/model/engine.py
@@ -147,7 +147,7 @@
   name: str
   fwd: G.Geom
   dgrad: Optional[G.Geom]
-  wf: t.Tensor
+  wf: Optional[t.Tensor]
   wd: Optional[t.Tensor]
   bias: t.Tensor
   gwf: t.Tensor
@@ -159,6 +159,7 @@
   ct_f: Optional[t.Tensor] = None
   ct_d: Optional[t.Tensor] = None
   ct_kind: str = ""
+  wf_ref: bool = False
 
 
 @dataclasses.dataclass(slots=True, eq=False)
@@ -208,7 +209,7 @@
 
   def __init__(self, num_classes: int, resolution=(128, 128, 128), latent_channels: int = 64,
                skip_fraction: float = 0.75, last_upscale_factor: int = 2, device="cuda",
-               backend=None, dtype=t.float32, decoder_math: Optional[str] = None):
+               backend=None, dtype=t.float32, decoder_math: Optional[str] = None, full_pack: bool = False):
     if tuple(resolution) != (128, 128, 128) or last_upscale_factor != 2:
       raise ValueError("the CoReNet decoder is only defined for resolution 128^3, "
                        "last_upscale_factor 2 (reconstruction_decoder.py:38-54,93-95)")
@@ -221,6 +222,7 @@
     if self.decoder_math not in ("fp32", "bf16x3"):
       raise ValueError(f"decoder_math must be 'fp32' or 'bf16x3', not {self.decoder_math!r}")
     self.encoder_e2d = self.decoder_math == "bf16x3"
+    self.full_pack = bool(full_pack)
     assert dtype == t.float32 or getattr(backend, "name", "") == "emu"
     self.dtype = dtype
     self.device = t.device(device)
@@ -358,7 +360,7 @@
       else:
         p = shape[-1] // 2
         add(name, G.conv_fwd(shape, p), G.conv_dgrad(shape, p))
-    idx_parts, sizes = [], []
+    idx_parts = []
     for name, fwd, dgrad, repeat, nref in reg:
       wo, bo = s.offset(name + "weight"), s.offset(name + "bias")
       def shift(ix, o):
@@ -369,30 +371,14 @@
                  and np.array_equal(dgrad.index, np.arange(len(dgrad.index))))
         parts.append(np.zeros(0, np.int64) if alias else shift(dgrad.index, wo))
       idx_parts.append(parts)
-    flat_len = sum(len(p) for parts in idx_parts for p in parts)
     assert max(int(p.max()) for parts in idx_parts for p in parts if len(p)) < 2 ** 31
-    self.packed = t.zeros(flat_len, dtype=self.dtype, device=self.device)
+    self._reg, self._idx_parts = reg, idx_parts
     gsize = sum(len(parts[0]) for parts in idx_parts)
     self.gpacked = t.zeros(gsize, dtype=self.dtype, device=self.device)
-    pack_parts, pack_is_bwd, pack_names, unpack_parts = [], [], [], []
-    po, go = 0, 0
+    unpack_parts, go = [], 0
     for (name, fwd, dgrad, repeat, nref), parts in zip(reg, idx_parts):
-      pack_parts.append((po, parts[0], fwd.npad, 0)); po += len(parts[0]); pack_is_bwd.append(False); pack_names.append(name)
-      pack_parts.append((po, parts[1], len(parts[1]), 0)); po += len(parts[1]); pack_is_bwd.append(False); pack_names.append(name)
-      if dgrad is not None and len(parts[2]):
-        pack_parts.append((po, parts[2], dgrad.npad, dgrad.taps if dgrad.taps > 1 else 0)); po += len(parts[2])
-        pack_is_bwd.append(True); pack_names.append(name)
       unpack_parts.append((go, parts[0], fwd.npad, 0)); go += len(parts[0])
-    dev = self._tiles_dev
-    self.pack_tiles = dev([pp for pp, bwd in zip(pack_parts, pack_is_bwd) if not bwd])
-    sel = lambda pred: [pp for pp, bwd, nm in zip(pack_parts, pack_is_bwd, pack_names) if not bwd and pred(nm)]
-    early = lambda nm: nm.startswith("encoder.stage1") or nm.startswith("encoder.stage2")
-    self.pack_tiles_enc = dev(sel(lambda nm: nm.startswith("encoder.")))
-    self.pack_tiles_enc_early = dev(sel(early))
-    self.pack_tiles_enc_late = dev(sel(lambda nm: nm.startswith("encoder.") and not early(nm)))
-    self.pack_tiles_dec = dev(sel(lambda nm: not nm.startswith("encoder.")))
-    self.pack_tiles_bwd = dev([pp for pp, bwd in zip(pack_parts, pack_is_bwd) if bwd])
-    self.unpack_tiles = dev(unpack_parts)
+    self.unpack_tiles = self._tiles_dev(unpack_parts)
     los = [min(o for k, (o, _) in s.off.items() if s.kind[k] == "param" and k.startswith(lb))
            for lb in GRAD_BUCKET_LABELS[:-1]] + [0]
     self.grad_buckets: List[Tuple[str, int, int]] = []
@@ -405,21 +391,15 @@
       self._bucket_tiles.append(sel)
       hi = lo
     self._bucket_dev = None
-    po, go = 0, 0
+    go = 0
     for (name, fwd, dgrad, repeat, nref), parts in zip(reg, idx_parts):
-      nwf, nb = len(parts[0]), len(parts[1])
-      wf = self.packed[po:po + nwf]; po += nwf
-      bias = self.packed[po:po + nb]; po += nb
-      wd = None
-      if dgrad is not None:
-        if len(parts[2]):
-          wd = self.packed[po:po + len(parts[2])]; po += len(parts[2])
-        else:
-          wd = s.view(name + "weight").view(-1)
-      gwf = self.gpacked[go:go + nwf]; go += nwf
-      self.convs[name] = Conv(name, fwd, dgrad, wf, wd, bias, gwf,
-                              s.view(name + "bias", grad=True), nref)
-    self._build_operands(reg, idx_parts)
+      gwf = self.gpacked[go:go + len(parts[0])]; go += len(parts[0])
+      self.convs[name] = Conv(name, fwd, dgrad, None, None, None, gwf, s.view(name + "bias", grad=True), nref)
+    self._build_ct_images()
+    self._packed_back = set()
+    self._retired = []
+    self.wop = None
+    self._build_packs()
 
   def _build_ct_images(self):
     self.ct_tables = {}
@@ -444,52 +424,136 @@
       setattr(self.convs[name], field, img)
       self.ct_tables[kind] = (t.as_tensor(tab, device=self.device), img)
 
-  def _build_operands(self, reg, idx_parts):
-    self.wop = None
-    self.op_tables = {}
-    self._build_ct_images()
+  def _image_layers(self):
+    img = {}
     if self.decoder_math != "bf16x3":
-      return
-    groups = {"enc_early": [], "enc_late": [], "dec": [], "bwd": []}
-    slices = []
-    po, eo = 0, 0
-    for (name, fwd, dgrad, repeat, nref), parts in zip(reg, idx_parts):
-      src_f = po; po += len(parts[0]) + len(parts[1])
-      src_d = po
-      if dgrad is not None:
-        po += len(parts[2])
+      return img
+    for (name, fwd, dgrad, repeat, nref), parts in zip(self._reg, self._idx_parts):
       if (name, "fwd") in BF16X3_LAUNCHES:
-        groups["dec"].append((src_f, eo, fwd, True))
-        slices.append((name, "wop_f", eo, G.slab_entries(fwd))); eo += G.slab_entries(fwd)
-        groups["bwd"].append((src_d, eo, dgrad, True))
-        slices.append((name, "wop_d", eo, G.slab_entries(dgrad))); eo += G.slab_entries(dgrad)
-        self.convs[name].wop_kind = "slab"
+        img[(name, "f")] = ("dec", True)
+        img[(name, "d")] = ("bwd", True)
         continue
       if not self.encoder_e2d or not name.startswith("encoder.") or name.startswith("encoder.stage1"):
         continue
-      self.convs[name].wop_kind = "e2d"
       if fwd.window != (1, 3, 3):
         continue
       if G.operand_eligible(fwd) and name[len("encoder.stage")] in "45":
-        groups["enc_early" if name.startswith("encoder.stage2") else "enc_late"].append((src_f, eo, fwd))
-        slices.append((name, "wop_f", eo, G.operand_entries(fwd))); eo += G.operand_entries(fwd)
+        img[(name, "f")] = ("enc_early" if name.startswith("encoder.stage2") else "enc_late", False)
       if dgrad is not None and len(parts[2]) and G.operand_eligible(dgrad):
-        groups["bwd"].append((src_d, eo, dgrad))
-        slices.append((name, "wop_d", eo, G.operand_entries(dgrad))); eo += G.operand_entries(dgrad)
+        img[(name, "d")] = ("bwd", False)
+    return img
+
+  def _reads_reference_layout(self, name: str, fwd: G.Geom) -> bool:
+    if not name.startswith("encoder.stage") or name.startswith("encoder.stage1") or fwd.taps != 1:
+      return False
+    ref = np.arange(fwd.nout)[None, :] * fwd.cin + np.arange(fwd.cin)[:, None]
+    return (fwd.cin % 4 == 0 and self.store.offset(name + "weight") % 4 == 0
+            and np.array_equal(np.asarray(fwd.index).reshape(fwd.cin, fwd.npad)[:, :fwd.nout], ref))
+
+  def _build_packs(self):
+    s, be = self.store, self.be
+    lean_img = not self.full_pack and hasattr(be, "bf3_operands_slab")
+    lean_ref = not self.full_pack and hasattr(be, "conv_fwd_nk")
+    images = self._image_layers()
+    direct = {k for k in images if lean_img and k not in self._packed_back}
+    pack_parts, pack_is_bwd, pack_names, where = [], [], [], {}
+    po = 0
+    for (name, fwd, dgrad, repeat, nref), parts in zip(self._reg, self._idx_parts):
+      ref = lean_ref and (name, "f") not in self._packed_back and self._reads_reference_layout(name, fwd)
+      rf = rb = rd = None
+      if not ref and (name, "f") not in direct:
+        pack_parts.append((po, parts[0], fwd.npad, 0)); pack_is_bwd.append(False); pack_names.append(name)
+        rf = (po, po + len(parts[0])); po += len(parts[0])
+      pack_parts.append((po, parts[1], len(parts[1]), 0)); pack_is_bwd.append(False); pack_names.append(name)
+      rb = (po, po + len(parts[1])); po += len(parts[1])
+      if dgrad is not None and len(parts[2]) and (name, "d") not in direct:
+        pack_parts.append((po, parts[2], dgrad.npad, dgrad.taps if dgrad.taps > 1 else 0)); pack_is_bwd.append(True)
+        pack_names.append(name)
+        rd = (po, po + len(parts[2])); po += len(parts[2])
+      where[name] = (rf, rb, rd, ref)
+    if getattr(self, "packed", None) is not None:
+      self._retired.append(self.packed)
+    self.packed = t.zeros(po, dtype=self.dtype, device=self.device)
+    dev = self._tiles_dev
+    self.pack_tiles = dev([pp for pp, bwd in zip(pack_parts, pack_is_bwd) if not bwd])
+    sel = lambda pred: [pp for pp, bwd, nm in zip(pack_parts, pack_is_bwd, pack_names) if not bwd and pred(nm)]
+    early = lambda nm: nm.startswith("encoder.stage1") or nm.startswith("encoder.stage2")
+    self.pack_tiles_enc = dev(sel(lambda nm: nm.startswith("encoder.")))
+    self.pack_tiles_enc_early = dev(sel(early))
+    self.pack_tiles_enc_late = dev(sel(lambda nm: nm.startswith("encoder.") and not early(nm)))
+    self.pack_tiles_dec = dev(sel(lambda nm: not nm.startswith("encoder.")))
+    self.pack_tiles_bwd = dev([pp for pp, bwd in zip(pack_parts, pack_is_bwd) if bwd])
+    for (name, fwd, dgrad, repeat, nref), parts in zip(self._reg, self._idx_parts):
+      rf, rb, rd, ref = where[name]
+      cv = self.convs[name]
+      cv.wf = s.view(name + "weight").view(-1) if ref else (self.packed[rf[0]:rf[1]] if rf else None)
+      cv.wf_ref = bool(ref)
+      cv.bias = self.packed[rb[0]:rb[1]]
+      cv.wd = None
+      if dgrad is not None:
+        if not len(parts[2]):
+          cv.wd = s.view(name + "weight").view(-1)
+        elif rd:
+          cv.wd = self.packed[rd[0]:rd[1]]
+    self._lean_keys = direct | {(name, "f") for name, w in where.items() if w[3]}
+    self._build_operands(images, direct, where)
+
+  def require_packed(self, keys):
+    new = {k for k in keys if k in self._lean_keys}
+    if not new:
+      return
+    self._packed_back |= new
+    for p in self.plans.values():
+      p.graphs, p.eval_graph, p.eval_eager, p.eager_steps = {}, None, 0, 0
+    self._build_packs()
+    self.weights_dirty = True
+
+  def _build_operands(self, images, direct, where):
+    self.op_tables, self.op_slab_tables = {}, {}
+    for cv in self.convs.values():
+      cv.wop_f = cv.wop_d = None
+      cv.wop_kind = ""
+    groups = {"enc_early": [], "enc_late": [], "dec": [], "bwd": []}
+    groups_direct = {k: [] for k in groups}
+    slices = []
+    eo = 0
+    for name, fwd, dgrad, repeat, nref in self._reg:
+      if (name, "fwd") in BF16X3_LAUNCHES and self.decoder_math == "bf16x3":
+        self.convs[name].wop_kind = "slab"
+      elif self.encoder_e2d and name.startswith("encoder.") and not name.startswith("encoder.stage1"):
+        self.convs[name].wop_kind = "e2d"
+      for d, g, field in (("f", fwd, "wop_f"), ("d", dgrad, "wop_d")):
+        if (name, d) not in images:
+          continue
+        group, slab = images[(name, d)]
+        n = G.slab_entries(g) if slab else G.operand_entries(g)
+        if (name, d) in direct:
+          groups_direct[group].append((self.store.offset(name + "weight"), eo, g, slab))
+        else:
+          groups[group].append((where[name][0 if d == "f" else 2][0], eo, g, slab))
+        slices.append((name, field, eo, n)); eo += n
     if not eo:
       return
-    self.wop = t.zeros(eo * 32, dtype=t.uint8, device=self.device)
+    if self.wop is None:
+      self.wop = t.zeros(eo * 32, dtype=t.uint8, device=self.device)
     for name, field, e0, n in slices:
       setattr(self.convs[name], field, self.wop[e0 * 32:(e0 + n) * 32])
     for k, layers in groups.items():
       if layers:
         desc, blocks = G.operand_table(layers)
         self.op_tables[k] = (t.as_tensor(desc, device=self.device), blocks)
+    for k, layers in groups_direct.items():
+      if layers:
+        desc, blocks, table, lds = G.operand_slab_table(layers)
+        self.op_slab_tables[k] = (t.as_tensor(desc, device=self.device), blocks,
+                                  None if table is None else t.as_tensor(table, device=self.device), lds)
 
   def _operands(self, *groups):
     for k in groups:
       if k in self.op_tables:
         self.be.bf3_operands(self.packed, self.op_tables[k], self.wop)
+      if k in self.op_slab_tables:
+        self.be.bf3_operands_slab(self.store.params, self.op_slab_tables[k], self.wop)
       if k in self.ct_tables:
         self.be.bf3_gather_image(self.store.params, *self.ct_tables[k])
 
@@ -639,6 +703,7 @@
                              gv1=f(B, ci, r, r, r), gv2=f(B, cm, r, r, r))
     self.logits = f(B, C, 128, 128, 128)
     self.glogits = f(B, C, 128, 128, 128)
+    eng.require_packed(self._needs_packed())
     self.skip_src = {2: "stage5", 3: "stage4", 4: "stage3", 5: "stage2"}
     self.skip_hw = {k: stage_hw[self.skip_src[k]] for k in self.skip_src}
     self.smap = {k: f(B, self.skip_hw[k][0], self.skip_hw[k][1], sk[k]) for k in sk}
@@ -670,6 +735,26 @@
     self._skip_bwd_done = t.cuda.Event() if use_side else None
     self._skip_async_live = False
 
+  def _needs_packed(self):
+    eng, keys = self.eng, set()
+    cur = self.p1
+    for blk in self.blocks:
+      p = blk.prefix
+      cb = eng.convs[p + "op_b.conv."]
+      if cb.wop_kind == "e2d" and not self._e2d_shape_ok(self.vw(blk.yb), cb.fwd.window):
+        keys |= {(cb.name, "f"), (cb.name, "d")}
+      xin = self.vw(blk.xs if blk.stride == 2 else cur)
+      bb = eng.bns[p + "op_b.bn."]
+      calls = [("op_a.conv.", xin, None, blk.ya), ("op_c.conv.", self.vw(blk.yb), Transform(bb.scale, bb.shift, post_relu=True), blk.yc)]
+      if blk.down:
+        calls.append(("shortcut.conv.", xin, None, blk.ys))
+      for nm, xv, tr, y in calls:
+        cv = eng.convs[p + nm]
+        if cv.wf_ref and not self.be.conv_fwd_nk_ok(xv, tr, cv.wf, self.vw(y)):
+          keys.add((cv.name, "f"))
+      cur = blk.out
+    return keys
+
   def _cached(self, key, fn):
     v = self._views.get(key)
     if v is None:
@@ -770,9 +855,16 @@
       self._timed("fwd   " + cv.name, lambda: self.be.conv2d_bf3(
           x, tr, cv.wop_f, g.npad, cv.bias, 0, y, g.window, g.pad_lo, accumulate))
       return
+    if cv.wf_ref:
+      self._timed("fwd   " + cv.name, lambda: self.be.conv_fwd_nk(x, tr, cv.wf, cv.bias, 0, y, accumulate))
+      return
+    math = self._math(cv, "fwd")
+    wslab = cv.wop_f if cv.wop_kind == "slab" else None
+    if cv.wf is None and not (math == "bf16x3" and wslab is not None):
+      raise RuntimeError(f"{cv.name}: this forward launch reads fp32 packed weights, which the engine does not pack for the layer")
     self._timed("fwd   " + cv.name, lambda: self.be.conv_fwd(
         x, tr, cv.wf, g.npad, cv.bias, 0, y, g.window, g.pad_lo, 0, accumulate, boxes=(g.n_boxes, g.c_boxes),
-        math=self._math(cv, "fwd"), wslab=cv.wop_f if cv.wop_kind == "slab" else None))
+        math=math, wslab=wslab))
 
   def _dgrad(self, cv: Conv, dy: V.View, dx: V.View, accumulate=False):
     g = cv.dgrad
@@ -780,9 +872,13 @@
       self._timed("dgrad " + cv.name, lambda: self.be.conv2d_bf3(
           dy, None, cv.wop_d, g.npad, None, 0, dx, g.window, g.pad_lo, accumulate))
       return
+    math = self._math(cv, "dgrad")
+    wslab = cv.wop_d if cv.wop_kind == "slab" else None
+    if cv.wd is None and not (math == "bf16x3" and wslab is not None):
+      raise RuntimeError(f"{cv.name}: this data-gradient launch reads fp32 packed weights, which the engine does not pack for the layer")
     self._timed("dgrad " + cv.name, lambda: self.be.conv_fwd(
         dy, None, cv.wd, g.npad, None, 0, dx, g.window, g.pad_lo, 0, accumulate, boxes=(g.n_boxes, g.c_boxes),
-        math=self._math(cv, "dgrad"), wslab=cv.wop_d if cv.wop_kind == "slab" else None))
+        math=math, wslab=wslab))
 
   def _dgrad_bn_bwd(self, cv: Conv, dy: V.View, g: t.Tensor, x: t.Tensor, Cn: int, S: int, b, dx: t.Tensor, cprev: Conv) -> bool:
     be = self.be
diff --git a/include/corenet_hip.h b/include/corenet_hip.h
--- a/include/corenet_hip.h
+++ b/include/corenet_hip.h
@@ -40,6 +40,9 @@
                  int kd, int kh, int kw, int pd, int ph, int pw,
                  int splits, int accumulate ,
                  const crnTapBoxes* boxes , crnStream stream);
+int crn_conv_fwd_nk(const crnView* x, const crnInTransform* tr, const float* w, const float* bias, int bias_sB,
+                    const crnView* y, int accumulate, crnStream stream);
+int crn_conv_fwd_nk_plan(const crnView* x, const crnInTransform* tr, const float* w, const crnView* y);
 
 #define CRN_PLAN_DENSE_COLS 1
 #define CRN_PLAN_DENSE_ROWS 2
@@ -148,6 +151,8 @@
 
 int crn_bf3_operands(const float* packed, const int64_t* desc, int nlayers, int64_t total_blocks, void* out,
                      crnStream stream);
+int crn_bf3_operands_slab(const float* slab, const int64_t* desc, int nlayers, int64_t total_blocks, const int32_t* table,
+                          int lds_bytes, void* out, crnStream stream);
 int crn_conv2d_bf3(const crnView* x, const crnInTransform* tr, const void* wop, int Npad, const float* bias,
                    int bias_sB, const crnView* y, int kh, int kw, int ph, int pw, int accumulate, crnStream stream);
 
```
